# vita-epfl/Stable-Video-Infinity

Measured on AMD Instinct MI355X. Metric: denoised latent frames/sec, Wan2.1-1.3B 81f@832x480 50-step, higher is better.
Workload: dtype bf16

## Files before the change

include/svi_hip.h:

```cpp
#ifndef SVI_HIP_H
#define SVI_HIP_H

#include <stdint.h>

#ifdef __cplusplus
extern "C" {
#endif

#define SVI_HIP_ABI_VERSION 13

typedef enum {
    SVI_OK = 0,
    SVI_ERR_INVALID = 1,
    SVI_ERR_UNBOUND = 2,
    SVI_ERR_HIP = 3,
    SVI_ERR_UNSUPPORTED = 4,
    SVI_ERR_OOM = 5
} svi_status;

typedef enum { SVI_BF16 = 0, SVI_F32 = 1, SVI_F16 = 2 ,
               SVI_E4M3 = 3  } svi_dtype;

typedef void* svi_stream;
typedef struct svi_dit svi_dit;
// ... 32 lines not shown

svi_status svi_dit_forward(svi_dit* h, const void* x, const float* timestep, const void* context,
                           const void* clip_feature, const void* y, const void* add_condition,
                           void* out, int32_t B, int32_t T, int32_t H, int32_t W, int32_t Lc,
                           svi_stream stream);

svi_status svi_dit_set_audio(svi_dit* h, const void* audio_first, const void* audio_latter, int32_t n_latter);

svi_status svi_dit_audio_slot(svi_dit* h, int32_t slot , const void* audio_first, const void* audio_latter, int32_t n_latter,
                              svi_stream stream);
svi_status svi_dit_forward_talk3(svi_dit* h, const void* x, const float* timestep, const void* context_cond, const void* context_uncond,
                                 const void* clip_feature, const void* y, const void* add_condition, void* out_cond, void* out_uncond,
                                 void* out_drop_text, int32_t T, int32_t H, int32_t W, int32_t Lc, svi_stream stream);
svi_status svi_audio_windows(const void* emb, svi_dtype dtype, int32_t N, int32_t R, int32_t start, int32_t T_latent, void* first_out,
                             void* latter_out, svi_stream stream);
svi_status svi_dit_audio_slot_windows(svi_dit* h, int32_t slot , const void* emb, svi_dtype dtype, int32_t N, int32_t start,
                                      int32_t T_latent, svi_stream stream);
svi_status svi_dit_forward_talk3_tea(svi_dit* h, const void* x, const float* timestep, const void* context_cond, const void* context_uncond,
                                     const void* clip_feature, const void* y, const void* add_condition, void* out_cond, void* out_uncond,
                                     void* out_drop_text, int32_t T, int32_t H, int32_t W, int32_t Lc, int32_t tea_cond, int32_t tea_uncond,
                                     int32_t tea_drop_text, void* residual_cond, void* residual_uncond, void* residual_drop_text, svi_stream stream);

svi_status svi_dit_time_mod(svi_dit* h, const float* timestep, void* t_mod_out, int32_t B, svi_stream stream);
svi_status svi_dit_forward_tea(svi_dit* h, const void* x, const float* timestep, const void* context,
                               const void* clip_feature, const void* y, const void* add_condition, void* out,
                               int32_t B, int32_t T, int32_t H, int32_t W, int32_t Lc, int32_t tea_mode, void* residual,
                               svi_stream stream);

svi_status svi_dit_forward_cfg_pair(svi_dit* h, const void* x, const float* timestep, const void* context_cond,
                                    const void* context_uncond, const void* clip_feature, const void* y,
                                    const void* add_condition, void* out_cond, void* out_uncond, int32_t B, int32_t T,
                                    int32_t H, int32_t W, int32_t Lc, svi_stream stream);
svi_status svi_dit_forward_cfg_pair_tea(svi_dit* h, const void* x, const float* timestep, const void* context_cond,
                                        const void* context_uncond, const void* clip_feature, const void* y,
                                        const void* add_condition, void* out_cond, void* out_uncond, int32_t B, int32_t T,
                                        int32_t H, int32_t W, int32_t Lc, int32_t tea_mode, void* residual_cond, void* residual_uncond,
                                        svi_stream stream);

svi_status svi_dit_context_cache(svi_dit* h, int32_t enable);
svi_status svi_dit_context_refill(svi_dit* h, const void* context, const void* clip_feature, int32_t Lc, svi_stream stream);

svi_status svi_dit_sp_begin(svi_dit* h, const void* x, const float* timestep, const void* context, const void* clip_feature,
                            const void* y, const void* add_condition, int32_t T, int32_t H, int32_t W, int32_t Lc,
                            int32_t row0, int32_t nrows, svi_stream stream);
svi_status svi_dit_sp_begin_pair(svi_dit* h, const void* x, const float* timestep, const void* context_cond, const void* context_uncond,
                                 const void* clip_feature, const void* y, const void* add_condition, int32_t T, int32_t H, int32_t W, int32_t Lc,
                                 int32_t row0, int32_t nrows, svi_stream stream);
svi_status svi_dit_sp_block_qkv_part(svi_dit* h, int32_t layer, void* q_send, void* k_send, void* vt_out, int32_t ldvt, int32_t P, int32_t G,
                                     int32_t part, svi_stream stream);
svi_status svi_dit_sp_block_qkv(svi_dit* h, int32_t layer, void* q_send, void* k_send, void* vt_out, int32_t ldvt, int32_t P, int32_t G,
                                svi_stream stream);
svi_status svi_sp_unpack_vt(const void* recv, void* out, int32_t P, int32_t Dp, int32_t Ls, int32_t lds, int32_t L8, int32_t nb, int32_t Dg, svi_stream stream);
svi_status svi_sp_unpack_out(const void* recv, void* out, int32_t P, int32_t G, int32_t Ls, int32_t Dg, int32_t nb, svi_stream stream);
svi_status svi_dit_sp_block_rest(svi_dit* h, int32_t layer, const void* attn, svi_stream stream);
svi_status svi_dit_sp_tea(svi_dit* h, int32_t mode, void* residual, svi_stream stream);
svi_status svi_dit_sp_head(svi_dit* h, void* head_rows_out, svi_stream stream);
svi_status svi_dit_unpatchify(svi_dit* h, const void* head_rows, void* out, int32_t T, int32_t H, int32_t W, svi_stream stream);
int32_t svi_dit_head_ld(svi_dit* h);
int64_t svi_dit_generation(svi_dit* h);
svi_status svi_stream_buffers_release(svi_stream stream, int32_t all_streams);
svi_status svi_attention_vt_fwd(const void* q, int32_t ldq, const void* k, int32_t ldk, const void* vt, int32_t ldvt, void* out,
                                int32_t ldo, int32_t s_q, int32_t s_kv, int32_t n, int32_t q_prescaled, svi_stream stream);
svi_status svi_attention_frames_fwd(const void* q, int32_t ldq, const void* k, int32_t ldk, const void* vt, int32_t ldvt, void* out, int32_t ldo,
                                    int32_t row0, int32_t nrows, int32_t rows_per_frame, int32_t keys_per_frame, int32_t n, svi_stream stream);

svi_status svi_linear_row_stats(const void* A, int32_t lda, const void* W, int32_t ldw, void* C, int32_t ldc, int32_t M, int32_t N, int32_t K,
                                const void* bias, float eps, float* row_sumsq, int32_t ldss, float* rs_out, svi_stream stream);
svi_status svi_cross_attention_fwd(const void* q, int32_t ldq, const void* k, int32_t ldk, const void* vt, int32_t ldvt, void* out, int32_t ldo,
                                   int32_t s_q, int32_t s_kv, int32_t n, const int32_t* key_tail, const float* q_rs, const void* q_gain,
                                   float q_out_scale, svi_stream stream);

svi_status svi_dit_block_forward(svi_dit* h, int32_t layer, void* x_inout, const void* context,
                                 const void* t_mod, int32_t f, int32_t hh, int32_t ww, int32_t Lc,
                                 svi_stream stream);

svi_status svi_attention_fwd(const void* q, const void* k, const void* v, void* out, int32_t b,
                             int32_t s_q, int32_t s_kv, int32_t n, int32_t d, svi_stream stream);
svi_status svi_attention_last_flagged(svi_stream stream, int32_t* flagged_out, int32_t* workgroups_out);
svi_status svi_gemm_plan(int32_t M, int32_t N, int32_t K, int32_t epilogue, int32_t skinny, int32_t compute_units, int32_t* kernel_out);
svi_status svi_gemm_w8_plan(int32_t M, int32_t N, int32_t K, int32_t epilogue, int32_t skinny, int32_t compute_units, int32_t* kernel_out);
svi_status svi_attention_plan(int32_t s_q, int32_t s_kv, int32_t heads, int32_t compute_units, int32_t* out4);
svi_status svi_vae_conv_plan(int32_t Cin, int32_t Cout, int32_t kt, int32_t frames, int32_t Ho, int32_t Wo, int64_t* out8);
svi_status svi_vae_tile_order(int32_t ord_T, int32_t ord_Lf, int32_t ord_G, int64_t* out);

svi_status svi_layernorm_modulate(const void* x, void* out, int32_t rows, int32_t dim, float eps,
                                  const void* w, const void* b, const void* shift, const void* scale,
                                  svi_stream stream);

svi_status svi_rmsnorm_rope(void* x, int32_t ld, int32_t rows, int32_t dim, const void* weight, float eps,
                            int32_t rope, int32_t num_heads, int32_t f, int32_t h, int32_t w,
                            svi_stream stream);

svi_status svi_rmsnorm_rope_qk(void* x, int32_t ld, int32_t rows, int32_t dim, const void* weight_q, const void* weight_k,
                               float eps, float out_scale_q, float out_scale_k, int32_t rope,
                               int32_t f, int32_t h, int32_t w, int32_t row0, int32_t period, svi_stream stream);

svi_status svi_gemm_bf16(const void* A, int32_t lda, const void* W, int32_t ldw, void* C, int32_t ldc,
                         int32_t M, int32_t N, int32_t K, const void* bias, int32_t bias_along_m,
                         int32_t epilogue, const float* gate, const void* res, int32_t ldres,
                         svi_stream stream);
svi_status svi_gemm_bf16_pair(const void* A, int32_t lda, const void* W, int32_t ldw, void* C, int32_t ldc,
                              int32_t M, int32_t N, int32_t K, const void* bias, int32_t bias_along_m,
                              int32_t epilogue, const float* gate, const void* res, int32_t ldres,
                              const void* W2, const void* bias2, int32_t n_split, int32_t sel_m, int32_t sel_n,
                              svi_stream stream);
svi_status svi_gemm_bf16_skinny(const void* A, int32_t lda, const void* W, int32_t ldw, void* C, int32_t ldc, int32_t M, int32_t N, int32_t K,
                                const void* bias, int32_t epilogue, const float* gate, const void* res, int32_t ldres, int32_t w8, svi_stream stream);
svi_status svi_gemm_bf16_w8(const void* A, int32_t lda, const void* W8, int32_t ldw, void* C, int32_t ldc,
                            int32_t M, int32_t N, int32_t K, const void* bias, int32_t bias_along_m,
                            int32_t epilogue, const float* gate, const void* res, int32_t ldres,
                            const void* W2_8, const void* bias2, int32_t n_split, int32_t sel_m, int32_t sel_n,
                            svi_stream stream);

svi_status svi_mx8_quantize(const void* x, int32_t ldx, int32_t rows, int32_t K, void* q, int32_t ldq, void* scales, int32_t sc_rows, svi_stream stream);
svi_status svi_gemm_mx8(const void* A8, int32_t lda, const void* a_scales, int32_t sc_rows, const void* W8, int32_t ldw, void* C, int32_t ldc,
                        int32_t M, int32_t N, int32_t K, const void* bias, int32_t epilogue, const float* gate, const void* res, int32_t ldres,
                        svi_stream stream);
svi_status svi_dit_bind_ffn_fp8(svi_dit* h, int32_t layer, int32_t which, const void* e4m3_weight);
svi_status svi_dit_ffn_mx8(svi_dit* h, int32_t enable);
svi_status svi_gemm_mx8_wscaled(const void* A8, int32_t lda, const void* W8, int32_t ldw, const void* w_scales, int32_t sc_rows, void* C, int32_t ldc,
                                int32_t M, int32_t N, int32_t K, const void* bias, int32_t bias_along_m, svi_stream stream);
svi_status svi_dit_proj_mx8(svi_dit* h, int32_t enable);

svi_status svi_cfg_step(void* latents, const void* cond, const void* uncond, int64_t n, float cfg_scale,
                        float dsigma, svi_stream stream);

svi_status svi_cfg3_step(void* latents, const void* cond, const void* uncond, const void* drop_text, int64_t n, float s_text,
                         float s_audio, float dsigma, svi_stream stream);

svi_status svi_fp8_e4m3_to_bf16(const void* in, void* out, int64_t n, svi_stream stream);

svi_status svi_f32_to_fp8_e4m3(const void* in, svi_dtype in_dtype, void* out, int64_t n, svi_stream stream);

svi_status svi_lora_merge_e4m3(void* w8, int32_t out_f, int32_t in_f, const void* up, const void* down_t, svi_dtype dtype, int32_t r, float alpha,
                               svi_stream stream);

svi_status svi_prof_enable(int32_t on);
svi_status svi_prof_summary(char* buf, int64_t buflen);
svi_status svi_prof_select(const char* tags);

svi_status svi_vae_create(svi_vae** out);
svi_status svi_vae_destroy(svi_vae* h);
svi_status svi_vae_bind_weight(svi_vae* h, const char* name, const void* dev_ptr, svi_dtype dtype,
                               const int64_t* shape, int32_t rank);
svi_status svi_vae_check_bound(svi_vae* h);
svi_status svi_video_to_u8(const float* video, uint8_t* frames, int32_t T, int32_t H, int32_t W, svi_stream stream);
svi_status svi_u8_to_video(const uint8_t* frames, float* video, int32_t n, int32_t H, int32_t W, svi_stream stream);

svi_status svi_vae_decode(svi_vae* h, const float* latents, float* video, int32_t T, int32_t hh, int32_t ww,
                          svi_stream stream);
svi_status svi_vae_encode(svi_vae* h, const float* video, float* latents, int32_t T, int32_t H, int32_t W,
                          svi_stream stream);

svi_status svi_vae_tiled_decode(svi_vae* h, const float* latents, float* video, int32_t T, int32_t hh, int32_t ww,
                                int32_t size_h, int32_t size_w, int32_t stride_h, int32_t stride_w, svi_stream stream);
svi_status svi_vae_tiled_encode(svi_vae* h, const float* video, float* latents, int32_t T, int32_t H, int32_t W,
                                int32_t size_h, int32_t size_w, int32_t stride_h, int32_t stride_w, svi_stream stream);

svi_status svi_vae_split_plan(int32_t hh, int32_t ww, int32_t parts_h, int32_t parts_w, int32_t part, int32_t* out24);
svi_status svi_vae_decode_part(svi_vae* h, const float* latents, float* video, int32_t T, int32_t hh, int32_t ww, int32_t parts_h, int32_t parts_w,
                               int32_t part, int32_t video_ld_h, int32_t video_ld_w, svi_stream stream);
svi_status svi_vae_decode_planned(svi_vae* h, const float* latents, float* video, int32_t T, int32_t hh, int32_t ww, const int32_t* plan24,
                                  int32_t video_ld_h, int32_t video_ld_w, svi_stream stream);

svi_status svi_vae_encode_split_plan(int32_t hh, int32_t ww, int32_t parts_h, int32_t parts_w, int32_t part, int32_t* out34);
svi_status svi_vae_encode_part(svi_vae* h, const float* video, float* feat_out, int32_t T, int32_t H, int32_t W, int32_t parts_h, int32_t parts_w,
// ... 63 lines not shown
```

stable-video-infinity_amd/csrc/svi_api.hip:

```cpp
#include <algorithm>
#include <string>
#include <stdlib.h>
#include <string.h>
#include <atomic>
#include <deque>
#include <mutex>
#include <vector>

#include "svi_common.h"

static thread_local char g_err[512] = "";

void svi_set_error(const char* fmt, ...) {
    va_list ap;
    va_start(ap, fmt);
    vsnprintf(g_err, sizeof(g_err), fmt, ap);
    va_end(ap);
}

extern "C" const char* svi_last_error(void) { return g_err; }

static int env_int(const char* name, int lo, int dflt) {
    const char* v = getenv(name);
    if (!v || !*v) return dflt;
    char* end = nullptr;
    const long x = strtol(v, &end, 10);
    if (end == v || x < lo || x > (1 << 20)) { fprintf(stderr, "libsvi_hip: ignoring %s=%s (expected an integer >= %d)\n", name, v, lo); return dflt; }
    return (int)x;
}
static SviSwitches parse_switches() {
    SviSwitches s;
    s.flash_kernel = env_int("SVI_FLASH_KERNEL", 1, 0);
    if (s.flash_kernel > 2) s.flash_kernel = 0;
    s.gemm_kernel = env_int("SVI_GEMM_KERNEL", 128, 0);
    if (s.gemm_kernel != 128 && s.gemm_kernel != 192 && s.gemm_kernel != 259 && s.gemm_kernel != 260) {
        if (s.gemm_kernel != 0)
            fprintf(stderr, "libsvi_hip: ignoring SVI_GEMM_KERNEL=%d (kernels: 128, 192, 259 = 256^2 four phases, 260 = 256^2 two phases; 256 / 257 / 258 are retired)\n", s.gemm_kernel);
        s.gemm_kernel = 0;
    }
    s.gemm_gm = env_int("SVI_GEMM_GM", 1, 0);
    s.gemm_pf = env_int("SVI_GEMM_PF", 1, 0);
    if (s.gemm_pf != 0 && s.gemm_pf != 1 && s.gemm_pf != 4 && s.gemm_pf != 8) s.gemm_pf = 0;
    s.vae_exact_fp32 = getenv("SVI_VAE_EXACT_FP32") != nullptr;
    s.flash_two_pass = env_int("SVI_FLASH_TWO_PASS", 0, 1);
    s.flash_m16 = env_int("SVI_FLASH_M16", 0, 1);
    s.vae_no_x2h = env_int("SVI_VAE_X2H", 0, 1) == 0;
    s.cross_dedup = env_int("SVI_CROSS_DEDUP", 0, 1);
    s.cross_fused = env_int("SVI_CROSS_FUSED", 0, 1);
    s.vae_dma = env_int("SVI_VAE_DMA", 0, 1);
    s.vae_up_phases = env_int("SVI_VAE_UP_PHASES", 0, 1);
    s.vae_tile_order = env_int("SVI_VAE_TILE_ORDER", 0, 1);
    s.vae_pair = env_int("SVI_VAE_PAIR", 0, 1);
    s.mx8_fused = env_int("SVI_MX8_FUSED", 0, 1);
    s.qk_fused = env_int("SVI_QK_FUSED", 0, 1);
    s.attn_qk8 = env_int("SVI_ATTN_QK8", 0, 0) != 0;
    s.qk8_fused = env_int("SVI_QK8_FUSED", 0, 1);
    s.rms_rows = env_int("SVI_RMS_ROWS", 0, 1);
    s.flash_split = env_int("SVI_FLASH_SPLIT", 0, 0);
    if (s.flash_split > 4) s.flash_split = 4;
    s.ws_limit_mb = env_int("SVI_WS_LIMIT_MB", 1, 0);
    { const char* v = getenv("SVI_T5_BUCKETS"); s.t5_host_buckets = v && strcmp(v, "host") == 0; }
    return s;
}
static std::atomic<const SviSwitches*>& switches_ptr() {
    static std::atomic<const SviSwitches*> p{new SviSwitches(parse_switches())};
    return p;
}
const SviSwitches& svi_switches() { return *switches_ptr().load(std::memory_order_acquire); }
static std::atomic<unsigned long long> g_stream_buffer_generation{0};
extern "C" svi_status svi_switches_reload(void) {
    switches_ptr().store(new SviSwitches(parse_switches()), std::memory_order_release);
    g_stream_buffer_generation.fetch_add(1, std::memory_order_relaxed);
    return SVI_OK;
}

extern "C" int32_t svi_switch_state(const char* name) {
    if (!name) return -1;
    const SviSwitches& sw = svi_switches();
    const std::string n(name);
    if (n == "SVI_ATTN_QK8") return sw.attn_qk8 ? 1 : 0;
    if (n == "SVI_CROSS_FUSED") return sw.cross_fused ? 1 : 0;
    if (n == "SVI_CROSS_DEDUP") return sw.cross_dedup ? 1 : 0;
    if (n == "SVI_QK_FUSED") return sw.qk_fused ? 1 : 0;
    if (n == "SVI_FLASH_TWO_PASS") return sw.flash_two_pass ? 1 : 0;
    if (n == "SVI_FLASH_M16") return sw.flash_m16 ? 1 : 0;
    return -1;
}

int svi_current_device() {
    int d = -1;
    if (hipGetDevice(&d) != hipSuccess) { (void)hipGetLastError(); svi_set_error("no usable HIP device"); return -1; }
    return d;
}

svi_status svi_claim_device(int* handle_device) {
    const int d = svi_current_device();
    if (d < 0) return SVI_ERR_HIP;
    if (*handle_device < 0) *handle_device = d;
    if (*handle_device != d) {
        svi_set_error("handle belongs to device %d but the current device is %d (one handle per device)", *handle_device, d);
        return SVI_ERR_INVALID;
    }
    return SVI_OK;
}

static std::mutex& table_mutex() {
    static std::mutex m;
    return m;
}

svi_status svi_ensure_lds(const void* kernel, int bytes) {
    struct Seen { int dev; const void* fn; };
    static std::vector<Seen> seen;
    const int dev = svi_current_device();
    if (dev < 0) return SVI_ERR_HIP;
    std::lock_guard<std::mutex> lock(table_mutex());
    for (const Seen& s : seen)
        if (s.dev == dev && s.fn == kernel) return SVI_OK;
    SVI_CHECK_HIP(hipFuncSetAttribute(kernel, hipFuncAttributeMaxDynamicSharedMemorySize, bytes));
    seen.push_back(Seen{dev, kernel});
    return SVI_OK;
}

namespace {
struct StreamSlot { int dev, kind; hipStream_t st; void* p; size_t bytes; long user; };
std::deque<StreamSlot>& stream_slots() {
    static std::deque<StreamSlot> slots;
    return slots;
}
}
unsigned long long svi_stream_buffer_generation() { return g_stream_buffer_generation.load(std::memory_order_relaxed); }

extern "C" svi_status svi_stream_buffers_release(svi_stream stream, int32_t all_streams) {
    const int dev = svi_current_device();
    if (dev < 0) return SVI_ERR_HIP;
// ... 339 lines not shown
    g.C = reinterpret_cast<bf16*>(C); g.ldc = ldc; g.M = M; g.N = N; g.K = K;
    g.bias = reinterpret_cast<const bf16*>(bias); g.bias_along_m = bias_along_m; g.epi = epilogue; g.gate = gate;
    g.res = reinterpret_cast<const bf16*>(res); g.ldres = ldres;
    if (W2) { g.W2 = reinterpret_cast<const bf16*>(W2); g.bias2 = reinterpret_cast<const bf16*>(bias2); g.n_split = n_split; }
    g.sel_m = sel_m; g.sel_n = sel_n;
    return svi_launch_gemm_e8(g, 1, reinterpret_cast<hipStream_t>(stream));
}

extern "C" svi_status svi_gemm_bf16_skinny(const void* A, int32_t lda, const void* W, int32_t ldw, void* C, int32_t ldc, int32_t M, int32_t N, int32_t K,
                                           const void* bias, int32_t epilogue, const float* gate, const void* res, int32_t ldres, int32_t w8, svi_stream stream) {
    SVI_REQUIRE(A && W && C, "svi_gemm_bf16_skinny: null argument");
    SviGemmArgs g{};
    g.A = reinterpret_cast<const bf16*>(A); g.lda = lda; g.W = reinterpret_cast<const bf16*>(W); g.ldw = ldw;
    g.C = reinterpret_cast<bf16*>(C); g.ldc = ldc; g.M = M; g.N = N; g.K = K;
    g.bias = reinterpret_cast<const bf16*>(bias); g.epi = epilogue; g.gate = gate; g.res = reinterpret_cast<const bf16*>(res); g.ldres = ldres;
    g.skinny = 1;
    SVI_REQUIRE(svi_gemm_choose(g, 256) == 0, "svi_gemm_bf16_skinny: M = %d, K = %d, epilogue %d do not take the skinny kernel (M <= 128, K %% 128 == 0, bias or gate + residual)", M, K, epilogue);
    return w8 ? svi_launch_gemm_e8(g, 1, reinterpret_cast<hipStream_t>(stream)) : svi_launch_gemm(g, reinterpret_cast<hipStream_t>(stream));
}

extern "C" svi_status svi_linear_row_stats(const void* A, int32_t lda, const void* W, int32_t ldw, void* C, int32_t ldc, int32_t M, int32_t N, int32_t K,
                                           const void* bias, float eps, float* row_sumsq, int32_t ldss, float* rs_out, svi_stream stream) {
    SVI_REQUIRE(A && W && C && row_sumsq && rs_out, "svi_linear_row_stats: null argument");
    SVI_REQUIRE(N > 0 && N % 64 == 0 && ldss >= M, "svi_linear_row_stats: N = %d must be a multiple of 64 and ldss >= M", N);
    hipStream_t st = reinterpret_cast<hipStream_t>(stream);
    SviGemmArgs g{};
    g.A = reinterpret_cast<const bf16*>(A); g.lda = lda; g.W = reinterpret_cast<const bf16*>(W); g.ldw = ldw;
    g.C = reinterpret_cast<bf16*>(C); g.ldc = ldc; g.M = M; g.N = N; g.K = K;
    g.bias = reinterpret_cast<const bf16*>(bias); g.epi = SVI_EPI_BIAS;
    g.rowss = row_sumsq; g.ldss = ldss;
    SVI_TRY(svi_launch_gemm(g, st));
    return svi_launch_row_rs(row_sumsq, N / 64, ldss, M, N, eps, rs_out, st);
}
extern "C" svi_status svi_cross_attention_fwd(const void* q, int32_t ldq, const void* k, int32_t ldk, const void* vt, int32_t ldvt, void* out, int32_t ldo,
                                              int32_t s_q, int32_t s_kv, int32_t n, const int32_t* key_tail, const float* q_rs, const void* q_gain,
                                              float q_out_scale, svi_stream stream) {
    SVI_REQUIRE(q && k && vt && out, "svi_cross_attention_fwd: null argument");
    SVI_REQUIRE(s_q > 0 && s_kv > 0 && n > 0 && ldq >= n * 128 && ldk >= n * 128 && ldo >= n * 128 && ldvt >= s_kv, "svi_cross_attention_fwd: bad sizes");
    SVI_REQUIRE((q_rs == nullptr) == (q_gain == nullptr), "svi_cross_attention_fwd: q_rs and q_gain come together");
    hipStream_t st = reinterpret_cast<hipStream_t>(stream);
    SviProfScope _p(PROF_FLASH_CROSS, st);
    const SviQNorm qn{q_rs, reinterpret_cast<const bf16*>(q_gain), q_out_scale};
    int key_blocks = 0;
    if (key_tail) {
        hipStreamCaptureStatus cs = hipStreamCaptureStatusNone;
        int n = 0;
        if (hipStreamIsCapturing(st, &cs) == hipSuccess && cs == hipStreamCaptureStatusNone &&
            hipMemcpyAsync(&n, key_tail, sizeof(int), hipMemcpyDeviceToHost, st) == hipSuccess && hipStreamSynchronize(st) == hipSuccess && n > 0)
            key_blocks = (std::min(n, s_kv) + 31) / 32;
        else (void)hipGetLastError();
    }
    return svi_launch_flash_cross(reinterpret_cast<const bf16*>(q), ldq, reinterpret_cast<const bf16*>(k), ldk, reinterpret_cast<const bf16*>(vt), ldvt,
                                  reinterpret_cast<bf16*>(out), ldo, s_q, s_kv, n, st, key_tail, q_rs ? &qn : nullptr, key_blocks);
}

extern "C" svi_status svi_gemm_plan(int32_t M, int32_t N, int32_t K, int32_t epilogue, int32_t skinny, int32_t compute_units, int32_t* kernel_out) {
    SVI_REQUIRE(kernel_out && M > 0 && N > 0 && K > 0 && compute_units > 0, "svi_gemm_plan: bad argument");
    SviGemmArgs g{};
    g.M = M; g.N = N; g.K = K; g.lda = K; g.ldw = K; g.ldc = (N + 7) / 8 * 8; g.epi = epilogue; g.skinny = skinny;
    *kernel_out = svi_gemm_choose(g, compute_units);
    return SVI_OK;
}
extern "C" svi_status svi_gemm_w8_plan(int32_t M, int32_t N, int32_t K, int32_t epilogue, int32_t skinny, int32_t compute_units, int32_t* kernel_out) {
    SVI_REQUIRE(kernel_out && M > 0 && N > 0 && K > 0 && compute_units > 0, "svi_gemm_w8_plan: bad argument");
    SviGemmArgs g{};
    g.M = M; g.N = N; g.K = K; g.lda = K; g.ldw = K; g.ldc = (N + 7) / 8 * 8; g.epi = epilogue; g.skinny = skinny;
    *kernel_out = svi_gemm_choose_e8(g, compute_units, 1);
    return SVI_OK;
}
extern "C" svi_status svi_attention_plan(int32_t s_q, int32_t s_kv, int32_t heads, int32_t compute_units, int32_t* out4) {
    SVI_REQUIRE(out4 && s_q > 0 && s_kv > 0 && heads > 0 && compute_units > 0, "svi_attention_plan: bad argument");
    int kernel = 0;
    const SviFlashSplit sp = svi_flash_plan(s_q, s_kv, heads, compute_units, &kernel);
    const int items = sp.qblocks * sp.heads;
    out4[0] = kernel; out4[1] = sp.whole; out4[2] = sp.pieces; out4[3] = sp.whole + (items - sp.whole) * sp.pieces;
    return SVI_OK;
}
extern "C" svi_status svi_vae_conv_plan(int32_t Cin, int32_t Cout, int32_t kt, int32_t frames, int32_t Ho, int32_t Wo, int64_t* out8) {
    return svi_vae_conv_choose(Cin, Cout, kt, frames, Ho, Wo, out8);
}
extern "C" svi_status svi_vae_tile_order(int32_t ord_T, int32_t ord_Lf, int32_t ord_G, int64_t* out) {
    return svi_vae_tile_order_fill(ord_T, ord_Lf, ord_G, out);
}

extern "C" svi_status svi_mx8_quantize(const void* x, int32_t ldx, int32_t rows, int32_t K, void* q, int32_t ldq, void* scales, int32_t sc_rows,
                                       svi_stream stream) {
    SVI_REQUIRE(x && q && scales, "svi_mx8_quantize: null argument");
    return svi_launch_mx8_quantize(reinterpret_cast<const bf16*>(x), ldx, rows, K, reinterpret_cast<unsigned char*>(q), ldq, reinterpret_cast<unsigned*>(scales), sc_rows,
                                   reinterpret_cast<hipStream_t>(stream));
}
extern "C" svi_status svi_gemm_mx8(const void* A8, int32_t lda, const void* a_scales, int32_t sc_rows, const void* W8, int32_t ldw, void* C, int32_t ldc,
                                   int32_t M, int32_t N, int32_t K, const void* bias, int32_t epilogue, const float* gate, const void* res, int32_t ldres,
                                   svi_stream stream) {
    SVI_REQUIRE(A8 && a_scales && W8 && C, "svi_gemm_mx8: null argument");
    SviGemmArgs g{};
    g.A = reinterpret_cast<const bf16*>(A8); g.lda = lda; g.W = reinterpret_cast<const bf16*>(W8); g.ldw = ldw;
    g.C = reinterpret_cast<bf16*>(C); g.ldc = ldc; g.M = M; g.N = N; g.K = K;
    g.bias = reinterpret_cast<const bf16*>(bias); g.epi = epilogue; g.gate = gate; g.res = reinterpret_cast<const bf16*>(res); g.ldres = ldres;
    return svi_launch_gemm_mx8(g, reinterpret_cast<const unsigned*>(a_scales), sc_rows, reinterpret_cast<hipStream_t>(stream));
}

extern "C" svi_status svi_gemm_mx8_wscaled(const void* A8, int32_t lda, const void* W8, int32_t ldw, const void* w_scales, int32_t sc_rows, void* C, int32_t ldc,
                                           int32_t M, int32_t N, int32_t K, const void* bias, int32_t bias_along_m, svi_stream stream) {
    SVI_REQUIRE(A8 && w_scales && W8 && C, "svi_gemm_mx8_wscaled: null argument");
    SviGemmArgs g{};
    g.A = reinterpret_cast<const bf16*>(A8); g.lda = lda; g.W = reinterpret_cast<const bf16*>(W8); g.ldw = ldw;
    g.C = reinterpret_cast<bf16*>(C); g.ldc = ldc; g.M = M; g.N = N; g.K = K;
    g.bias = reinterpret_cast<const bf16*>(bias); g.bias_along_m = bias_along_m; g.epi = SVI_EPI_BIAS;
    return svi_launch_gemm_mx8_wscaled(g, reinterpret_cast<const unsigned*>(w_scales), sc_rows, reinterpret_cast<hipStream_t>(stream));
}

extern "C" svi_status svi_cfg_step(void* latents, const void* cond, const void* uncond, int64_t n, float cfg_scale,
                                   float dsigma, svi_stream stream) {
    SVI_REQUIRE(latents && cond, "svi_cfg_step: null argument");
    return svi_launch_cfg_step(reinterpret_cast<bf16*>(latents), reinterpret_cast<const bf16*>(cond),
                               reinterpret_cast<const bf16*>(uncond), n, cfg_scale, dsigma,
                               reinterpret_cast<hipStream_t>(stream));
}

extern "C" svi_status svi_fp8_e4m3_to_bf16(const void* in, void* out, int64_t n, svi_stream stream) {
    SVI_REQUIRE(in && out && n >= 0, "svi_fp8_e4m3_to_bf16: bad argument");
    return svi_launch_fp8_e4m3_to_bf16(reinterpret_cast<const unsigned char*>(in), reinterpret_cast<bf16*>(out), n, reinterpret_cast<hipStream_t>(stream));
}

extern "C" svi_status svi_cfg3_step(void* latents, const void* cond, const void* uncond, const void* drop_text, int64_t n, float s_text,
                                    float s_audio, float dsigma, svi_stream stream) {
    SVI_REQUIRE(latents && cond && uncond && drop_text && n >= 0, "svi_cfg3_step: bad argument");
    return svi_launch_cfg3_step(reinterpret_cast<bf16*>(latents), reinterpret_cast<const bf16*>(cond), reinterpret_cast<const bf16*>(uncond),
                                reinterpret_cast<const bf16*>(drop_text), n, s_text, s_audio, dsigma, reinterpret_cast<hipStream_t>(stream));
}

extern "C" svi_status svi_audio_windows(const void* emb, svi_dtype dtype, int32_t N, int32_t R, int32_t start, int32_t T_latent, void* first_out,
                                        void* latter_out, svi_stream stream) {
    SVI_REQUIRE(emb, "svi_audio_windows: emb is NULL");
    SVI_REQUIRE(dtype == SVI_F32 || dtype == SVI_BF16, "svi_audio_windows: emb must be fp32 or bf16 (dtype %d)", (int)dtype);
    SVI_REQUIRE(N >= 1, "svi_audio_windows: N = %d audio frames (at least one)", N);
    SVI_REQUIRE(T_latent >= 1, "svi_audio_windows: T_latent = %d (at least one latent frame)", T_latent);
    SVI_REQUIRE(R > 0 && R % 8 == 0, "svi_audio_windows: R = %d must be a positive multiple of 8", R);
    SVI_REQUIRE(start >= 0, "svi_audio_windows: start = %d is negative", start);
    SVI_REQUIRE(first_out && (T_latent == 1 || latter_out), "svi_audio_windows: NULL output");
    if (svi_current_device() < 0) return SVI_ERR_HIP;
    return svi_launch_audio_windows(emb, dtype == SVI_F32, N, R, start, T_latent, reinterpret_cast<bf16*>(first_out), reinterpret_cast<bf16*>(latter_out),
                                    reinterpret_cast<hipStream_t>(stream));
}
```

stable-video-infinity_amd/csrc/svi_common.h:

```cpp
#pragma once

#include <hip/hip_runtime.h>
#include <stdint.h>
#include <stdarg.h>
#include <stdio.h>

#include "../../include/svi_hip.h"

typedef __bf16 bf16;
typedef __attribute__((ext_vector_type(8))) __bf16 bf16x8;
typedef __attribute__((ext_vector_type(4))) __bf16 bf16x4;
typedef __attribute__((ext_vector_type(2))) __bf16 bf16x2;
typedef __attribute__((ext_vector_type(16))) float f32x16;
typedef __attribute__((ext_vector_type(4))) float f32x4;
typedef __attribute__((ext_vector_type(4))) unsigned int u32x4;
typedef __attribute__((ext_vector_type(2))) unsigned int u32x2;

#define SVI_WAVE 64

void svi_set_error(const char* fmt, ...);

#define SVI_CHECK_HIP(expr)                                                                   \
    do {                                                                                      \
        hipError_t _e = (expr);                                                               \
        if (_e != hipSuccess) {                                                               \
            svi_set_error("%s failed: %s (%s:%d)", #expr, hipGetErrorString(_e), __FILE__, __LINE__); \
            return SVI_ERR_HIP;                                                               \
        }                                                                                     \
    } while (0)

#define SVI_REQUIRE(cond, ...)                                                                \
    do {                                                                                      \
        if (!(cond)) {                                                                        \
            svi_set_error(__VA_ARGS__);                                                       \
            return SVI_ERR_INVALID;                                                           \
        }                                                                                     \
    } while (0)

#define SVI_LAUNCH_CHECK()                                                                    \
    do {                                                                                      \
        hipError_t _e = hipGetLastError();                                                    \
        if (_e != hipSuccess) {                                                               \
            svi_set_error("kernel launch failed: %s (%s:%d)", hipGetErrorString(_e), __FILE__, __LINE__); \
            return SVI_ERR_HIP;                                                               \
        }                                                                                     \
    } while (0)

#define SVI_TRY(expr)                                                                         \
    do {                                                                                      \
        svi_status _s = (expr);                                                               \
        if (_s != SVI_OK) return _s;                                                          \
    } while (0)

struct SviSwitches {
    int flash_kernel = 0;
    int gemm_kernel = 0;
    int gemm_pf = 0;
    int gemm_gm = 0;
    int vae_exact_fp32 = 0;
    int vae_no_x2h = 0;
    int vae_dma = 1;
    int vae_pair = 1;
    int vae_tile_order = 1;
    int vae_up_phases = 1;
    int flash_two_pass = 1;
    int flash_m16 = 1;
    int flash_split = 0;
    int rms_rows = 1;
    int qk_fused = 1;
    int mx8_fused = 1;
    int attn_qk8 = 0;
    int qk8_fused = 1;
    int cross_fused = 1;
    int cross_dedup = 1;
    int t5_host_buckets = 0;
    int ws_limit_mb = 0;
};
const SviSwitches& svi_switches();

svi_status svi_ensure_lds(const void* kernel, int bytes);
enum SviBufKind { SVI_BUF_FLASH_FLAGS = 0, SVI_BUF_SEAM_SCRATCH = 1, SVI_BUF_SEAM_SMALL = 2, SVI_BUF_FLASH_SPLIT = 3, SVI_BUF_FLASH_QK8 = 4 };
svi_status svi_stream_buffer(int kind, hipStream_t st, size_t bytes, void** out, long** user_out);
int svi_current_device();
svi_status svi_claim_device(int* handle_device);
#define SVI_REQUIRE_DEVICE(h) SVI_TRY(svi_claim_device(&(h)->device))

#ifdef __HIPCC__
__device__ __forceinline__ float rbf(float v) { return (float)(bf16)v; }

__device__ __forceinline__ float wave_sum(float v) {
#pragma unroll
    for (int o = 32; o > 0; o >>= 1) v += __shfl_xor(v, o);
    return v;
}
__device__ __forceinline__ float wave_max(float v) {
#pragma unroll
    for (int o = 32; o > 0; o >>= 1) v = fmaxf(v, __shfl_xor(v, o));
    return v;
}

__device__ __forceinline__ bf16x8 ld_bf16x8(const bf16* p) { return *reinterpret_cast<const bf16x8*>(p); }
__device__ __forceinline__ void st_bf16x8(bf16* p, bf16x8 v) { *reinterpret_cast<bf16x8*>(p) = v; }

__device__ __forceinline__ void mx8_quant8(const float (&v)[8], bool live, int row, int c8, unsigned char* __restrict__ q, int ldq,
                                           unsigned* __restrict__ scales, int sc_rows) {
    float amax = 0.f;
#pragma unroll
    for (int e = 0; e < 8; ++e) amax = fmaxf(amax, fabsf(v[e]));
    amax = fmaxf(amax, __shfl_xor(amax, 1));
    amax = fmaxf(amax, __shfl_xor(amax, 2));
    const int eb = (int)((__float_as_uint(amax) >> 23) & 0xffu);
    const int E = max(eb - 8, 0);
    const float inv = __uint_as_float((unsigned)(254 - E) << 23);
    unsigned w[2];
#pragma unroll
    for (int h2 = 0; h2 < 2; ++h2) {
        float a[4];
#pragma unroll
        for (int e = 0; e < 4; ++e) {
            const float t = v[4 * h2 + e] * inv;
            a[e] = t != t ? t : fminf(fmaxf(t, -448.f), 448.f);
        }
        unsigned pk = 0;
        pk = __builtin_amdgcn_cvt_pk_fp8_f32(a[0], a[1], pk, false);
        pk = __builtin_amdgcn_cvt_pk_fp8_f32(a[2], a[3], pk, true);
        w[h2] = pk;
    }
    if (live) *reinterpret_cast<u32x2*>(q + (size_t)row * ldq + c8 * 8) = u32x2{w[0], w[1]};
    const int lane = threadIdx.x & 63;
    const unsigned e0 = (unsigned)E;
    const unsigned e1 = (unsigned)__shfl(E, (lane & ~15) + 4), e2 = (unsigned)__shfl(E, (lane & ~15) + 8), e3 = (unsigned)__shfl(E, (lane & ~15) + 12);
    if (live && (lane & 15) == 0) scales[(size_t)(c8 >> 4) * sc_rows + row] = e0 | (e1 << 8) | (e2 << 16) | (e3 << 24);
}

__device__ __forceinline__ float gelu_tanh_f(float x) {
    const float A = -2.0f * 1.4426950408889634f * 0.7978845608028654f * 0.044715f, B = -2.0f * 1.4426950408889634f * 0.7978845608028654f;
    const float a = x * __builtin_fmaf(x * x, A, B);
    return x * __builtin_amdgcn_rcpf(1.0f + __builtin_amdgcn_exp2f(a));
}
__device__ __forceinline__ float gelu_erf_f(float x) { return 0.5f * x * (1.0f + erff(x * 0.7071067811865476f)); }
__device__ __forceinline__ float silu_f(float x) { return x / (1.0f + __expf(-x)); }
#endif

enum SviProfTag {
    PROF_LN = 0, PROF_GEMM_QKV, PROF_RMS_ROPE, PROF_FLASH_SELF, PROF_GEMM_O, PROF_GEMM_CROSS, PROF_FLASH_CROSS,
    PROF_GEMM_FFN1, PROF_GEMM_FFN2, PROF_EMBED, PROF_HEAD, PROF_VAE_CONV, PROF_VAE_OTHER, PROF_NTAGS
};
extern bool g_svi_prof_on;
extern unsigned g_svi_prof_mask;
void svi_prof_begin_impl(int tag, hipStream_t st);
void svi_prof_end_impl(int tag, hipStream_t st);
struct SviProfScope {
    int tag; hipStream_t st; bool on;
    SviProfScope(int t, hipStream_t s) : tag(t), st(s), on(g_svi_prof_on && ((g_svi_prof_mask >> t) & 1u)) { if (on) svi_prof_begin_impl(tag, st); }
    ~SviProfScope() { if (on) svi_prof_end_impl(tag, st); }
};

struct SviGemmArgs {
    const bf16* A; int lda;
    const bf16* W; int ldw;
    bf16* C; int ldc;
    int M, N, K;
    const bf16* bias; int bias_along_m;
    int epi;
    const float* gate;
    const bf16* res; int ldres;
    int sel_m, sel_n;
    int skinny;
    unsigned char* q8; int ldq8; unsigned* q8s; int q8_sc_rows;
    const bf16* W2; const bf16* bias2; int n_split;
    float* rowss; int ldss;
};
unsigned long long svi_stream_buffer_generation();
svi_status svi_launch_gemm(const SviGemmArgs& g, hipStream_t st);
int svi_gemm_choose(const SviGemmArgs& g, int compute_units);
svi_status svi_launch_gemm_e8(const SviGemmArgs& g, int e8, hipStream_t st);
int svi_gemm_choose_e8(const SviGemmArgs& g, int compute_units, int e8);
struct SviFlashSplit { int whole, pieces, qblocks, heads; };
SviFlashSplit svi_flash_plan(int Lq, int Lk, int heads, int cus, int* kernel_out);
svi_status svi_vae_conv_choose(int Cin, int Cout, int kt, int frames, int Ho, int Wo, int64_t* out8);
svi_status svi_vae_tile_order_fill(int ord_T, int ord_Lf, int ord_G, int64_t* out);
svi_status svi_launch_mx8_quantize(const bf16* x, int ldx, int rows, int K, unsigned char* q, int ldq, unsigned* scales, int sc_rows, hipStream_t st);
svi_status svi_launch_gemm_mx8(const SviGemmArgs& g, const unsigned* a_scales, int sc_rows, hipStream_t st);
svi_status svi_launch_gemm_mx8_wscaled(const SviGemmArgs& g, const unsigned* w_scales, int sc_rows, hipStream_t st);

#define SVI_QK_SCALE_LOG2E 0.12751743f
struct SviQk8 { unsigned char* q8; unsigned char* k8; unsigned* qs; unsigned* ks; int ld8, qs_rows, ks_rows; };
svi_status svi_launch_flash(const bf16* Q, int ldq, const bf16* K, int ldk, const bf16* VT, int ldvt,
                            bf16* O, int ldo, int Lq, int Lk, int num_heads, int q_prescaled, hipStream_t st, const int* key_tail = nullptr, const SviQk8* qk8 = nullptr);
svi_status svi_launch_flash_frames(const bf16* Q, int ldq, const bf16* K, int ldk, const bf16* VT, int ldvt, bf16* O, int ldo, int row0, int nrows,
                                   int rows_per_frame, int keys_per_frame, int num_heads, hipStream_t st);
struct SviQNorm { const float* rs; const bf16* gain; float out_scale; };
svi_status svi_launch_flash_cross(const bf16* Q, int ldq, const bf16* K, int ldk, const bf16* VT, int ldvt, bf16* O, int ldo, int Lq, int Lk, int num_heads,
                                  hipStream_t st, const int* key_tail, const SviQNorm* norm, int key_blocks = 0);
svi_status svi_launch_row_rs(const float* rowss, int groups, int ldss, int rows, int dim, float eps, float* rs, hipStream_t st);
svi_status svi_flash_qk8_prepare(int Lq, int Lk, int num_heads, hipStream_t st, SviQk8* out, bool* use, int batch = 1);
inline SviQk8 svi_qk8_sample(const SviQk8& b, int s, int Lq, int Lk) {
    SviQk8 v = b;
    v.q8 += (size_t)s * Lq * b.ld8; v.k8 += (size_t)s * Lk * b.ld8; v.qs += (size_t)s * Lq; v.ks += (size_t)s * Lk;
    return v;
}

svi_status svi_launch_ln_mod(const bf16* x, int ldx, bf16* out, int ldo, int rows, int dim, float eps,
                             const bf16* w, const bf16* b, const float* shift, const float* scale1p,
                             hipStream_t st);
struct SviRope {
    const float2* tab_f; const float2* tab_h; const float2* tab_w;
    int npf, nph, npw;
    int f, h, w;
    int row0;
    int period;
    const float2* tab_tok;
};
svi_status svi_launch_rope_token_table(const SviRope& r, float2* out, int tokens, hipStream_t st);
struct SviScatter { bf16* out0; bf16* out1; int P, Dp, Dg; int rows_per_sample; };
svi_status svi_launch_rmsnorm_rope(bf16* x, int ld, int rows, int dim, const bf16* weight, float eps,
                                   const SviRope* rope, float out_scale, hipStream_t st);
svi_status svi_launch_rmsnorm_rope2(bf16* x, int ld, int rows, int dim, const bf16* weight, const bf16* weight1, float eps,
                                    const SviRope* rope, float out_scale, float out_scale1, hipStream_t st, const SviScatter* scatter = nullptr);
bool svi_rmsnorm_rope_q8_ok(int dim, const SviRope* rope);
svi_status svi_launch_rmsnorm_rope2_q8(bf16* x, int ld, int rows, int dim, const bf16* weight, const bf16* weight1, float eps, const SviRope* rope, float out_scale,
                                       float out_scale1, hipStream_t st, const SviQk8& out);
svi_status svi_launch_sp_unpack_vt(const bf16* recv, bf16* out, int P, int Dp, int Ls, int lds, int L8, hipStream_t st, int nb = 1, int Dg = 0);
svi_status svi_launch_sp_unpack_out(const bf16* recv, bf16* out, int P, int G, int Ls, int Dg, hipStream_t st, int nb = 1);
svi_status svi_launch_transpose(const bf16* in, int ldi, bf16* out, int ldo, int rows, int cols, hipStream_t st);
svi_status svi_launch_cfg_step(bf16* lat, const bf16* cond, const bf16* uncond, int64_t n, float s, float dsigma,
                               hipStream_t st);
svi_status svi_launch_add_bf16(bf16* a_inout, const bf16* b, int64_t n, hipStream_t st);
svi_status svi_launch_cfg3_step(bf16* lat, const bf16* cond, const bf16* uncond, const bf16* drop, int64_t n, float st, float sa, float dsigma,
                                hipStream_t stream);
svi_status svi_launch_video_to_u8(const float* video, unsigned char* out, long thw, hipStream_t st);
svi_status svi_launch_u8_to_video(const unsigned char* frames, float* out, int n, long hw, hipStream_t st);
svi_status svi_launch_sub_bf16(bf16* out, const bf16* a, const bf16* b, int64_t n, hipStream_t st);
svi_status svi_launch_audio_windows(const void* emb, bool f32, int N, int R, int start, int T, bf16* first, bf16* latter, hipStream_t st);
svi_status svi_launch_add_ln_mod_pair(const bf16* x, const bf16* res_a, const bf16* res_b, bf16* out_a, bf16* out_b, int rows, int dim, float eps,
                                      const float* shift, const float* scale1p, hipStream_t st);
svi_status svi_launch_sub_sum_bf16(bf16* out, const bf16* a, const bf16* b, const bf16* c, int64_t n, hipStream_t st);
svi_status svi_launch_add_ln_mod_talk3(const bf16* x, const bf16* add_condition, const bf16* const res[3], bf16* const out[3], const bool with_addc[3],
                                       int rows, int dim, float eps, const float* shift, const float* scale1p, hipStream_t st);
svi_status svi_launch_fp8_e4m3_to_bf16(const unsigned char* in, bf16* out, int64_t n, hipStream_t st);
svi_status svi_launch_gemm_f32(const float* A, int lda, const float* W, int ldw, const float* bias, float* C, int ldc, int M, int N, int K,
                               const float* res, int ldres, hipStream_t st);
```

stable-video-infinity_amd/csrc/svi_vae.hip:

```cpp
#include <algorithm>
#include <map>
#include <string>
#include <vector>
#include <math.h>
#include <stdlib.h>
#include <string.h>

#include "svi_common.h"

namespace {

struct ConvP {
    const float* in; int Ti, Hi, Wi, Cin, ld_in;
    const float* w; int ld_w;
    const bf16* w3; int ld_w3; long plane_w3;
    const void* w2h; const float* w2_inv;
    float in_scale;
    const float* bias;
    float* out; int To, Ho, Wo, Cout, ld_out;
    int kt, kh, kw, st, sh, sw, pt, ph, pw;
    int ups;
    int zero_frame0;
    int t_begin;
    int out_mode;
    int pad_;
    int t_out_off;
    const float* res; int ld_res;
    int act_silu;
    bf16* out_bf16;
    const unsigned short* in_h; const unsigned short* in_l;
    int ord_T, ord_Lf, ord_G;
    int up_phase;
};

__device__ __forceinline__ int tile_off(int row, int chunk) { return row * 128 + ((chunk ^ ((row >> 1) & 7)) << 4); }

template <int NT>
__global__ __launch_bounds__(256, 2) void conv_igemm_kernel(ConvP p) {
    constexpr int A_BYTES = 128 * 128;
    constexpr int W_BYTES = NT * 32 * 128;
    extern __shared__ __attribute__((aligned(16))) char smem[];
    const int tid = threadIdx.x, lane = tid & 63, wave = tid >> 6;
    const int l31 = lane & 31, hi = lane >> 5;
    const long HoWo = (long)p.Ho * p.Wo;
    const long P_total = (long)p.To * HoWo;
    const long p0 = (long)p.t_begin * HoWo + (long)blockIdx.x * 128;
    const int co0 = blockIdx.y * 32 * NT;
    const int Hv = p.ups ? 2 * p.Hi : p.Hi, Wv = p.ups ? 2 * p.Wi : p.Wi;

    const int ld_chunk = tid & 7;
    int a_t[4], a_y[4], a_x[4];
    bool a_ok[4];
#pragma unroll
    for (int j = 0; j < 4; ++j) {
        const long pp = p0 + (tid >> 3) + 32 * j;
        a_ok[j] = pp < P_total;
        const long q = a_ok[j] ? pp : 0;
        a_t[j] = (int)(q / HoWo);
        const int rem = (int)(q - (long)a_t[j] * HoWo);
        a_y[j] = rem / p.Wo;
        a_x[j] = rem - a_y[j] * p.Wo;
    }
    const int nchunk = (p.Cin + 31) >> 5;
    const int ntaps = p.kt * p.kh * p.kw;
    const int nk = ntaps * nchunk;
    f32x4 ra[4], rw[NT];
    const f32x4 zero4 = {0.f, 0.f, 0.f, 0.f};

    auto load_tile = [&](int kidx) {
        const int tap = kidx / nchunk, cc = kidx - tap * nchunk;
        const int ta = tap / (p.kh * p.kw), tb = (tap / p.kw) % p.kh, tc = tap % p.kw;
        const int c = cc * 32 + ld_chunk * 4;
        const bool cin = c < p.Cin;
#pragma unroll
        for (int j = 0; j < 4; ++j) {
            const int ti = a_t[j] * p.st + ta - p.pt;
            int yi = a_y[j] * p.sh + tb - p.ph, xi = a_x[j] * p.sw + tc - p.pw;
            bool ok = a_ok[j] && cin && ti >= 0 && ti < p.Ti && yi >= 0 && yi < Hv && xi >= 0 && xi < Wv;
            if (p.zero_frame0 && ti == 0) ok = false;
            if (p.ups) { yi >>= 1; xi >>= 1; }
            ra[j] = ok ? *reinterpret_cast<const f32x4*>(p.in + (((long)ti * p.Hi + yi) * p.Wi + xi) * p.ld_in + c) : zero4;
        }
#pragma unroll
        for (int j = 0; j < NT; ++j) {
            const int co = co0 + (tid >> 3) + 32 * j;
            rw[j] = (cin && co < p.Cout) ? *reinterpret_cast<const f32x4*>(p.w + ((long)tap * p.Cout + co) * p.ld_w + c) : zero4;
        }
    };
    auto store_tile = [&](int buf) {
        char* As = smem + buf * (A_BYTES + W_BYTES);
        char* Ws = As + A_BYTES;
#pragma unroll
        for (int j = 0; j < 4; ++j) *reinterpret_cast<f32x4*>(As + tile_off((tid >> 3) + 32 * j, ld_chunk)) = ra[j];
#pragma unroll
        for (int j = 0; j < NT; ++j) *reinterpret_cast<f32x4*>(Ws + tile_off((tid >> 3) + 32 * j, ld_chunk)) = rw[j];
    };

    f32x16 acc[NT];
#pragma unroll
    for (int n = 0; n < NT; ++n)
#pragma unroll
        for (int r = 0; r < 16; ++r) acc[n][r] = 0.f;

    load_tile(0);
    store_tile(0);
    __syncthreads();
    for (int k = 0; k < nk; ++k) {
        const int cur = k & 1;
        if (k + 1 < nk) load_tile(k + 1);
        const char* As = smem + cur * (A_BYTES + W_BYTES);
        const char* Ws = As + A_BYTES;
#pragma unroll
        for (int q = 0; q < 4; ++q) {
            const f32x4 av = *reinterpret_cast<const f32x4*>(As + tile_off(32 * wave + l31, 2 * q + hi));
            f32x4 bv[NT];
// ... 366 lines not shown
    for (int k = 0; k < nk; k += 2) {
        SVI_X3_STEP(0, 0, k + 2, k + 2 < nk, 1, 1);
        __syncthreads();
        SVI_X3_STEP(1, 1, k + 3, k + 3 < nk, 0, 0);
        __syncthreads();
    }
#undef SVI_X3_STEP
#undef SVI_X3_ADVANCE
#undef SVI_X3_TAP_BASES
#undef SVI_X3_LOAD_A
#undef SVI_X3_LOAD_W
#undef SVI_X3_STAGE_A
#undef SVI_X3_STAGE_W
#undef SVI_X3_SPLIT1
#undef SVI_X3_MFMA
#undef SVI_X3_STORES
#undef SVI_X3_LOADS

    const long pp = p0 + 32 * wave + l31;
    if (pp >= P_total) return;
    const f32x4 zero4 = {0.f, 0.f, 0.f, 0.f};
    f32x4 bv[12], rv[12], sv[12];
    const bool with_res = p.out_mode == 0 && p.res;
    const float inv_a = H2 ? 1.0f / p.in_scale : 1.0f;
    long po = pp + (long)p.t_out_off * HoWo;
    if (!H2 && p.up_phase) {
        const int ph_ = p.up_phase - 1;
        const int t = (int)(pp / HoWo);
        const int rem = (int)(pp - (long)t * HoWo);
        const int y = rem / p.Wo, x = rem - y * p.Wo;
        po = ((long)(t + p.t_out_off) * (2 * p.Ho) + 2 * y + (ph_ >> 1)) * (2 * p.Wo) + 2 * x + (ph_ & 1);
    }
#pragma unroll
    for (int i = 0; i < 12; ++i) {
        const int co = co0 + 32 * (i >> 2) + 8 * (i & 3) + 4 * hi;
        const bool ok = co < p.Cout;
        bv[i] = (ok && p.bias) ? *reinterpret_cast<const f32x4*>(p.bias + co) : zero4;
        rv[i] = (ok && with_res) ? *reinterpret_cast<const f32x4*>(p.res + po * p.ld_res + co) : zero4;
        if constexpr (H2) sv[i] = ok ? *reinterpret_cast<const f32x4*>(p.w2_inv + co) * inv_a : zero4;
    }
    long pq0 = 0;
    const int half = p.Cout >> 1;
    if (p.out_mode != 0) {
        const int t = (int)(pp / HoWo);
        const long sp = pp - (long)t * HoWo;
        pq0 = (long)(1 + 2 * (t - 1)) * HoWo + sp;
    }
#pragma unroll
    for (int i = 0; i < 12; ++i) {
        const int n = i >> 2, rg = i & 3;
        const int co = co0 + 32 * n + 8 * rg + 4 * hi;
        if (co >= p.Cout) continue;
        f32x4 v;
#pragma unroll
        for (int e = 0; e < 4; ++e) {
            float a = acc[n][4 * rg + e];
            if constexpr (H2) a *= sv[i][e];
            v[e] = (a + bv[i][e]) + rv[i][e];
        }
        if (p.out_mode == 0) {
            *reinterpret_cast<f32x4*>(p.out + po * p.ld_out + co) = v;
        } else {
            const int j = co >= half ? 1 : 0;
            *reinterpret_cast<f32x4*>(p.out + (pq0 + (long)j * HoWo) * p.ld_out + (co - j * half)) = v;
        }
    }
}


#define D2_ROWS 272
__host__ __device__ __forceinline__ long conv_tile_at(int ord_T, int ord_Lf, int ord_G, long tile) {
    if (ord_T <= 0) return tile;
    const long per_group = (long)ord_T * ord_G;
    const int full = ord_Lf / ord_G;
    const long g = tile / per_group;
    int gl = ord_G;
    long r = tile - g * per_group, gbase = g * ord_G;
    if (g >= full) { gl = ord_Lf - full * ord_G; r = tile - (long)full * per_group; gbase = (long)full * ord_G; }
    const int t = (int)(r / gl), j = (int)(r - (long)t * gl);
    return (long)t * ord_Lf + gbase + j;
}
#define D2_A_PLANE (D2_ROWS * 64)
#define D2_STAGE (2 * D2_A_PLANE + 6 * X3_W_PLANE)
template <int NB>
__global__ __launch_bounds__(512, 2) void conv_dma2h_kernel(ConvP p) {
#ifdef SVI_D2_DENSE
    p.ld_in = 32; p.ld_w3 = 32;
#endif
    constexpr int WP = 2 * NB;
    constexpr int NPIECE = 34 + 6 * WP;
    constexpr int D2_SLOTS = (NPIECE + 7) / 8;
    extern __shared__ __attribute__((aligned(16))) char smem[];
    const int tid = threadIdx.x, lane = tid & 63;
    const int wave = __builtin_amdgcn_readfirstlane(tid >> 6);
    const int l31 = lane & 31, hi = lane >> 5;
    const long HoWo = (long)p.Ho * p.Wo;
    const long P_total = (long)p.To * HoWo;
    const int ncob = (p.Cout + NB * 32 - 1) / (NB * 32);
    long tile = blockIdx.x / ncob;
    const int cob = (int)(blockIdx.x - tile * ncob);
    if (p.ord_T > 0) tile = conv_tile_at(p.ord_T, p.ord_Lf, p.ord_G, tile);
    const long p0 = (long)p.t_begin * HoWo + tile * X3_PIX;
    const int co0 = cob * NB * 32;
    const int nchunk = p.Cin >> 5;
    const int nrow = p.kt * p.kh;
    const int nk = nrow * nchunk;

    const int t_first = (int)(max(min(p0 - 1, P_total - 1), 0L) / HoWo);
    const int t_base = max(t_first * p.st - p.pt, 0);
    unsigned s_off[D2_SLOTS], s_mask[D2_SLOTS];
#pragma unroll
    for (int i = 0; i < D2_SLOTS; ++i) {
        const int q = wave + 8 * i;
        s_off[i] = 0xFFF00000u; s_mask[i] = 0;
        if (q < 34) {
            const int r16 = q % 17, row = r16 * 16 + (lane >> 2);
            const long pp = p0 - 1 + row;
            const bool pix = pp >= 0 && pp < P_total;
            const long qq = pix ? pp : 0;
            const int at = (int)(qq / HoWo);
            const int rem = (int)(qq - (long)at * HoWo);
            const int ay = rem / p.Wo, ax = rem - ay * p.Wo;
            const int bt = at * p.st - p.pt, by = ay - p.ph;
            unsigned m = 0;
            for (int rt = 0; rt < nrow; ++rt) {
                const int ta = rt / p.kh, tb = rt - ta * p.kh;
                const int ti = bt + ta, yi = by + tb;
                bool ok = pix && ti >= 0 && ti < p.Ti && yi >= 0 && yi < p.Hi;
                if (p.zero_frame0 && ti == 0) ok = false;
                if (ok) m |= 1u << rt;
            }
            s_mask[i] = m;
            const int chunk = (lane & 3) ^ ((row >> 2) & 3);
            s_off[i] = (unsigned)((((bt - t_base) * p.Hi + by) * p.Wi + ax) * p.ld_in) * 2u + (unsigned)chunk * 16u;
        } else if (q < NPIECE) {
            const int w = q - 34, tc = w / (2 * WP), pl = (w % (2 * WP)) / WP, row = (w % WP) * 16 + (lane >> 2);
            const int chunk = (lane & 3) ^ ((row >> 2) & 3);
            if (co0 + row < p.Cout) s_off[i] = (unsigned)((pl * p.plane_w3 + ((long)tc * p.Cout + co0 + row) * p.ld_w3 + chunk * 8) * 2);
        }
    }
    const long base_el = (long)t_base * p.Hi * p.Wi * p.ld_in;
    const long rem_bytes = ((long)p.Ti * p.Hi * p.Wi * p.ld_in - base_el) * 2;
    const int win = (int)(unsigned)min(rem_bytes, 0xFFE00000L);
    const __amdgpu_buffer_rsrc_t rs_h = __builtin_amdgcn_make_buffer_rsrc(const_cast<unsigned short*>(p.in_h + base_el), 0, win, 0x00020000);
    const __amdgpu_buffer_rsrc_t rs_l = __builtin_amdgcn_make_buffer_rsrc(const_cast<unsigned short*>(p.in_l + base_el), 0, win, 0x00020000);
    const __amdgpu_buffer_rsrc_t rs_w = __builtin_amdgcn_make_buffer_rsrc(const_cast<void*>(p.w2h), 0, (int)(unsigned)min((long)2 * p.plane_w3 * 2, 0xFFE00000L), 0x00020000);
    const unsigned OOB = 0xFFF00000u;
    bool left_ok, right_ok;
    {
        const long pp = min(p0 + 32 * wave + l31, P_total - 1);
        const int ax = (int)(pp % p.Wo);
        left_ok = ax > 0; right_ok = ax < p.Wo - 1;
    }

    int it_rt = 0, it_cc = 0, it_ta = 0, it_tb = 0;
    auto request = [&](int buf) {
        char* As = smem + buf * D2_STAGE;
        char* Ws = As + 2 * D2_A_PLANE;
        const unsigned d_act = (unsigned)(((it_ta * p.Hi + it_tb) * p.Wi) * p.ld_in) * 2u + (unsigned)it_cc * 64u;
        const unsigned d_w = (unsigned)((long)it_rt * p.kw * p.Cout * p.ld_w3 * 2) + (unsigned)it_cc * 64u;
#pragma unroll
        for (int i = 0; i < D2_SLOTS; ++i) {
            const int q = wave + 8 * i;
            if (q < 34) {
#ifdef SVI_D2_SKIP_A
                if (it_rt | it_cc) continue;
#endif
                const int pl = q / 17, r16 = q % 17;
                const unsigned off = ((s_mask[i] >> it_rt) & 1u) ? s_off[i] + d_act : OOB;
                if (pl == 0) __builtin_amdgcn_raw_ptr_buffer_load_lds(rs_h, (lptr_t)(As + r16 * 1024), 16, off, 0, 0, 0);
                else __builtin_amdgcn_raw_ptr_buffer_load_lds(rs_l, (lptr_t)(As + D2_A_PLANE + r16 * 1024), 16, off, 0, 0, 0);
            } else if (q < NPIECE) {
#ifdef SVI_D2_SKIP_W
                if (it_rt | it_cc) continue;
#endif
                const int w = q - 34, tc = w / (2 * WP), pl = (w % (2 * WP)) / WP, r16 = w % WP;
                const unsigned off = s_off[i] == OOB ? OOB : s_off[i] + d_w;
                __builtin_amdgcn_raw_ptr_buffer_load_lds(rs_w, (lptr_t)(Ws + (tc * 2 + pl) * X3_W_PLANE + r16 * 1024), 16, off, 0, 0, 0);
            }
        }
    };
    auto advance = [&]() {
        if (++it_cc == nchunk) {
            it_cc = 0; ++it_rt;
            if (++it_tb == p.kh) { it_tb = 0; ++it_ta; }
        }
    };

    f32x16 acc[NB];
#pragma unroll
    for (int n = 0; n < NB; ++n)
#pragma unroll
        for (int r = 0; r < 16; ++r) acc[n][r] = 0.f;

    request(0);
    advance();
    __syncthreads();
    const f16x8 zero8 = {(f16)0, (f16)0, (f16)0, (f16)0, (f16)0, (f16)0, (f16)0, (f16)0};
    for (int k = 0; k < nk; ++k) {
        const int cur = k & 1;
        if (k + 1 < nk) request(cur ^ 1);
        advance();
        const char* As = smem + cur * D2_STAGE;
        const char* Ws = As + 2 * D2_A_PLANE;
        f16x8 ah[2], al[2], wh[2][NB], wl[2][NB];
        auto frags = [&](int sidx, int set) {
            const int tc = sidx >> 1, ks = sidx & 1;
            const bool live = tc == 0 ? left_ok : tc == 2 ? right_ok : true;
            f16x8 h_ = *reinterpret_cast<const f16x8*>(As + x3_off(32 * wave + l31 + tc, 2 * ks + hi));
            f16x8 l_ = *reinterpret_cast<const f16x8*>(As + D2_A_PLANE + x3_off(32 * wave + l31 + tc, 2 * ks + hi));
            if (tc != 1) { h_ = live ? h_ : zero8; l_ = live ? l_ : zero8; }
            ah[set] = h_; al[set] = l_;
#pragma unroll
            for (int n = 0; n < NB; ++n) {
                wh[set][n] = *reinterpret_cast<const f16x8*>(Ws + (tc * 2) * X3_W_PLANE + x3_off(32 * n + l31, 2 * ks + hi));
                wl[set][n] = *reinterpret_cast<const f16x8*>(Ws + (tc * 2 + 1) * X3_W_PLANE + x3_off(32 * n + l31, 2 * ks + hi));
            }
        };
        frags(0, 0);
#pragma unroll
        for (int sidx = 0; sidx < 6; ++sidx) {
            const int set = sidx & 1;
            if (sidx + 1 < 6) frags(sidx + 1, set ^ 1);
#pragma unroll
            for (int n = 0; n < NB; ++n) acc[n] = __builtin_amdgcn_mfma_f32_32x32x16_f16(wl[set][n], ah[set], acc[n], 0, 0, 0);
#pragma unroll
            for (int n = 0; n < NB; ++n) acc[n] = __builtin_amdgcn_mfma_f32_32x32x16_f16(wh[set][n], al[set], acc[n], 0, 0, 0);
#pragma unroll
            for (int n = 0; n < NB; ++n) acc[n] = __builtin_amdgcn_mfma_f32_32x32x16_f16(wh[set][n], ah[set], acc[n], 0, 0, 0);
        }
        __syncthreads();
    }

    const long pp = p0 + 32 * wave + l31;
    if (pp >= P_total) return;
    const f32x4 zero4 = {0.f, 0.f, 0.f, 0.f};
    f32x4 bv[4 * NB], rv[4 * NB], sv[4 * NB];
    const bool with_res = p.out_mode == 0 && p.res;
    const float inv_a = 1.0f / p.in_scale;
    const long po = pp + (long)p.t_out_off * HoWo;
#pragma unroll
    for (int i = 0; i < 4 * NB; ++i) {
        const int co = co0 + 32 * (i >> 2) + 8 * (i & 3) + 4 * hi;
        const bool ok = co < p.Cout;
        if (NB == 1 && ok && co + 4 > p.Cout) {
            bv[i] = zero4; sv[i] = zero4; rv[i] = zero4;
            for (int e = 0; e < 4; ++e)
                if (co + e < p.Cout) {
                    if (p.bias) bv[i][e] = p.bias[co + e];
                    sv[i][e] = p.w2_inv[co + e] * inv_a;
                    if (with_res) rv[i][e] = p.res[po * p.ld_res + co + e];
                }
            continue;
        }
        bv[i] = (ok && p.bias) ? *reinterpret_cast<const f32x4*>(p.bias + co) : zero4;
        rv[i] = (ok && with_res) ? *reinterpret_cast<const f32x4*>(p.res + po * p.ld_res + co) : zero4;
        sv[i] = ok ? *reinterpret_cast<const f32x4*>(p.w2_inv + co) * inv_a : zero4;
    }
    long pq0 = 0;
    const int half = p.Cout >> 1;
    if (p.out_mode != 0) {
        const int t = (int)(pp / HoWo);
        const long sp = pp - (long)t * HoWo;
        pq0 = (long)(1 + 2 * (t - 1)) * HoWo + sp;
    }
#pragma unroll
    for (int i = 0; i < 4 * NB; ++i) {
        const int n = i >> 2, rg = i & 3;
        const int co = co0 + 32 * n + 8 * rg + 4 * hi;
        if (co >= p.Cout) continue;
        f32x4 v;
#pragma unroll
        for (int e = 0; e < 4; ++e) v[e] = (acc[n][4 * rg + e] * sv[i][e] + bv[i][e]) + rv[i][e];
        if (p.out_mode == 0) {
            *reinterpret_cast<f32x4*>(p.out + po * p.ld_out + co) = v;
        } else {
            const int j = co >= half ? 1 : 0;
            *reinterpret_cast<f32x4*>(p.out + (pq0 + (long)j * HoWo) * p.ld_out + (co - j * half)) = v;
        }
    }
}

#define D2P_W_STAGE (6 * X3_W_PLANE)
#define D2P_LDS (2 * D2P_W_STAGE + 2 * 2 * D2_A_PLANE)
__global__ __launch_bounds__(512, 2) void conv_dma2h_pair_kernel(ConvP p) {
    constexpr int NB = 3, WP = 2 * NB;
    constexpr int A_SLOTS = 5, W_SLOTS = 5;
    extern __shared__ __attribute__((aligned(16))) char smem[];
    char* const Wbuf = smem;
    char* const Sbuf = smem + 2 * D2P_W_STAGE;
    const int tid = threadIdx.x, lane = tid & 63;
    const int wave = __builtin_amdgcn_readfirstlane(tid >> 6);
    const int l31 = lane & 31, hi = lane >> 5;
    const long HoWo = (long)p.Ho * p.Wo;
    const long P_total = (long)p.To * HoWo;
    const int ncob = (p.Cout + NB * 32 - 1) / (NB * 32);
    const long pair = blockIdx.x / ncob;
    const int cob = (int)(blockIdx.x - pair * ncob);
    const int co0 = cob * NB * 32;
    const int nchunk = p.Cin >> 5;
    const int nrow = p.kt * p.kh;
    const int nk = nrow * nchunk;
    const unsigned OOB = 0xFFF00000u;

    long p0[2];
    int t_base[2];
#pragma unroll
    for (int s = 0; s < 2; ++s) {
        long tile = 2 * pair + s;
        if (tile < (long)p.ord_T * p.ord_Lf) tile = conv_tile_at(p.ord_T, p.ord_Lf, p.ord_G, tile);
        p0[s] = (long)p.t_begin * HoWo + tile * X3_PIX;
        const int t_first = (int)(max(min(p0[s] - 1, P_total - 1), 0L) / HoWo);
        t_base[s] = max(t_first * p.st - p.pt, 0);
    }
    unsigned a_off[2][A_SLOTS], a_mask[2][A_SLOTS], w_off[W_SLOTS];
#pragma unroll
    for (int s = 0; s < 2; ++s)
#pragma unroll
        for (int i = 0; i < A_SLOTS; ++i) {
            const int q = wave + 8 * i;
            a_off[s][i] = OOB; a_mask[s][i] = 0;
            if (q < 34) {
                const int r16 = q % 17, row = r16 * 16 + (lane >> 2);
                const long pp = p0[s] - 1 + row;
                const bool pix = pp >= 0 && pp < P_total;
                const long qq = pix ? pp : 0;
                const int at = (int)(qq / HoWo);
                const int rem = (int)(qq - (long)at * HoWo);
                const int ay = rem / p.Wo, ax = rem - ay * p.Wo;
                const int bt = at * p.st - p.pt, by = ay - p.ph;
                unsigned m = 0;
                for (int rt = 0; rt < nrow; ++rt) {
                    const int ta = rt / p.kh, tb = rt - ta * p.kh;
                    const int ti = bt + ta, yi = by + tb;
                    bool ok = pix && ti >= 0 && ti < p.Ti && yi >= 0 && yi < p.Hi;
                    if (p.zero_frame0 && ti == 0) ok = false;
                    if (ok) m |= 1u << rt;
                }
                a_mask[s][i] = m;
                const int chunk = (lane & 3) ^ ((row >> 2) & 3);
                a_off[s][i] = (unsigned)((((bt - t_base[s]) * p.Hi + by) * p.Wi + ax) * p.ld_in) * 2u + (unsigned)chunk * 16u;
            }
        }
#pragma unroll
    for (int i = 0; i < W_SLOTS; ++i) {
        const int w = wave + 8 * i;
        w_off[i] = OOB;
        if (w < 6 * WP) {
            const int tc = w / (2 * WP), pl = (w % (2 * WP)) / WP, row = (w % WP) * 16 + (lane >> 2);
            const int chunk = (lane & 3) ^ ((row >> 2) & 3);
            if (co0 + row < p.Cout) w_off[i] = (unsigned)((pl * p.plane_w3 + ((long)tc * p.Cout + co0 + row) * p.ld_w3 + chunk * 8) * 2);
        }
    }
    __amdgpu_buffer_rsrc_t rs_h[2], rs_l[2];
#pragma unroll
    for (int s = 0; s < 2; ++s) {
        const long base_el = (long)t_base[s] * p.Hi * p.Wi * p.ld_in;
        const long rem_bytes = ((long)p.Ti * p.Hi * p.Wi * p.ld_in - base_el) * 2;
        const int win = (int)(unsigned)min(rem_bytes, 0xFFE00000L);
        rs_h[s] = __builtin_amdgcn_make_buffer_rsrc(const_cast<unsigned short*>(p.in_h + base_el), 0, win, 0x00020000);
        rs_l[s] = __builtin_amdgcn_make_buffer_rsrc(const_cast<unsigned short*>(p.in_l + base_el), 0, win, 0x00020000);
    }
    const __amdgpu_buffer_rsrc_t rs_w = __builtin_amdgcn_make_buffer_rsrc(const_cast<void*>(p.w2h), 0, (int)(unsigned)min((long)2 * p.plane_w3 * 2, 0xFFE00000L), 0x00020000);
    bool left_ok[2], right_ok[2];
#pragma unroll
    for (int s = 0; s < 2; ++s) {
        const long pp = min(p0[s] + 32 * wave + l31, P_total - 1);
// ... 27 lines not shown
        char* Ws = Wbuf + wb * D2P_W_STAGE;
        const unsigned d_w = (unsigned)((long)rt * p.kw * p.Cout * p.ld_w3 * 2) + (unsigned)cc * 64u;
#pragma unroll
        for (int i = 0; i < W_SLOTS; ++i) {
            const int w = wave + 8 * i;
            if ((i < 2) != (half == 0) || w >= 6 * WP) continue;
            const int tc = w / (2 * WP), pl = (w % (2 * WP)) / WP, r16 = w % WP;
            const unsigned off = w_off[i] == OOB ? OOB : w_off[i] + d_w;
            __builtin_amdgcn_raw_ptr_buffer_load_lds(rs_w, (lptr_t)(Ws + (tc * 2 + pl) * X3_W_PLANE + r16 * 1024), 16, off, 0, 0, 0);
        }
    };

    f32x16 acc[2][NB];
#pragma unroll
    for (int s = 0; s < 2; ++s)
#pragma unroll
        for (int n = 0; n < NB; ++n)
#pragma unroll
            for (int r = 0; r < 16; ++r) acc[s][n][r] = 0.f;
    const f16x8 zero8 = {(f16)0, (f16)0, (f16)0, (f16)0, (f16)0, (f16)0, (f16)0, (f16)0};
    auto multiply = [&](auto sc, int wb) {
        constexpr int S = decltype(sc)::value;
        const char* As = Sbuf + S * 2 * D2_A_PLANE;
        const char* Ws = Wbuf + wb * D2P_W_STAGE;
        f16x8 ah[2], al[2], wh[2][NB], wl[2][NB];
        auto frags = [&](int sidx, int set) {
            const int tc = sidx >> 1, ks = sidx & 1;
            const bool live = tc == 0 ? left_ok[S] : tc == 2 ? right_ok[S] : true;
            f16x8 h_ = *reinterpret_cast<const f16x8*>(As + x3_off(32 * wave + l31 + tc, 2 * ks + hi));
            f16x8 l_ = *reinterpret_cast<const f16x8*>(As + D2_A_PLANE + x3_off(32 * wave + l31 + tc, 2 * ks + hi));
            if (tc != 1) { h_ = live ? h_ : zero8; l_ = live ? l_ : zero8; }
            ah[set] = h_; al[set] = l_;
#pragma unroll
            for (int n = 0; n < NB; ++n) {
                wh[set][n] = *reinterpret_cast<const f16x8*>(Ws + (tc * 2) * X3_W_PLANE + x3_off(32 * n + l31, 2 * ks + hi));
                wl[set][n] = *reinterpret_cast<const f16x8*>(Ws + (tc * 2 + 1) * X3_W_PLANE + x3_off(32 * n + l31, 2 * ks + hi));
            }
        };
        frags(0, 0);
#pragma unroll
        for (int sidx = 0; sidx < 6; ++sidx) {
            const int set = sidx & 1;
            if (sidx + 1 < 6) frags(sidx + 1, set ^ 1);
#pragma unroll
            for (int n = 0; n < NB; ++n) acc[S][n] = __builtin_amdgcn_mfma_f32_32x32x16_f16(wl[set][n], ah[set], acc[S][n], 0, 0, 0);
#pragma unroll
            for (int n = 0; n < NB; ++n) acc[S][n] = __builtin_amdgcn_mfma_f32_32x32x16_f16(wh[set][n], al[set], acc[S][n], 0, 0, 0);
#pragma unroll
            for (int n = 0; n < NB; ++n) acc[S][n] = __builtin_amdgcn_mfma_f32_32x32x16_f16(wh[set][n], ah[set], acc[S][n], 0, 0, 0);
        }
    };
    std::integral_constant<int, 0> T0;
    std::integral_constant<int, 1> T1;

    request_w(0, 0, 0, 0);
    request_w(1, 0, 0, 0);
    request_strip(T0, 0, 0, 0, 0);
    step_next(n_rt, n_cc, n_ta, n_tb);
    __syncthreads();
    for (int k = 0; k < nk; ++k) {
        const int wb = k & 1;
        const bool more = k + 1 < nk;
        request_strip(T1, c_rt, c_cc, c_ta, c_tb);
        if (more) request_w(0, n_rt, n_cc, wb ^ 1);
        multiply(T0, wb);
        __syncthreads();
        if (more) {
            request_strip(T0, n_rt, n_cc, n_ta, n_tb);
            request_w(1, n_rt, n_cc, wb ^ 1);
        }
        multiply(T1, wb);
        __syncthreads();
        step_next(c_rt, c_cc, c_ta, c_tb);
        step_next(n_rt, n_cc, n_ta, n_tb);
    }

    const f32x4 zero4 = {0.f, 0.f, 0.f, 0.f};
    const bool with_res = p.out_mode == 0 && p.res;
    const float inv_a = 1.0f / p.in_scale;
    const int half = p.Cout >> 1;
#pragma unroll
    for (int s = 0; s < 2; ++s) {
        const long pp = p0[s] + 32 * wave + l31;
        if (pp >= P_total) continue;
        const long po = pp + (long)p.t_out_off * HoWo;
        long pq0 = 0;
        if (p.out_mode != 0) {
            const int t = (int)(pp / HoWo);
            const long sp = pp - (long)t * HoWo;
            pq0 = (long)(1 + 2 * (t - 1)) * HoWo + sp;
        }
#pragma unroll
        for (int i = 0; i < 4 * NB; ++i) {
            const int n = i >> 2, rg = i & 3;
            const int co = co0 + 32 * n + 8 * rg + 4 * hi;
            if (co >= p.Cout) continue;
            const f32x4 bv = p.bias ? *reinterpret_cast<const f32x4*>(p.bias + co) : zero4;
            const f32x4 rv = with_res ? *reinterpret_cast<const f32x4*>(p.res + po * p.ld_res + co) : zero4;
            const f32x4 sv = *reinterpret_cast<const f32x4*>(p.w2_inv + co) * inv_a;
            f32x4 v;
#pragma unroll
            for (int e = 0; e < 4; ++e) v[e] = (acc[s][n][4 * rg + e] * sv[e] + bv[e]) + rv[e];
            if (p.out_mode == 0) {
                *reinterpret_cast<f32x4*>(p.out + po * p.ld_out + co) = v;
            } else {
                const int j = co >= half ? 1 : 0;
                *reinterpret_cast<f32x4*>(p.out + (pq0 + (long)j * HoWo) * p.ld_out + (co - j * half)) = v;
            }
        }
    }
}

bool conv_planes_ok(const ConvP& p) {
    const bool vec_ok = (((uintptr_t)p.w2_inv | (uintptr_t)p.bias) & 15) == 0;
    const bool wide = p.Cout >= 64 && p.Cout % 4 == 0 && vec_ok && (p.out_mode == 0 || (p.Cout / 2) % 4 == 0);
    const bool narrow = p.Cout <= 32 && p.out_mode == 0 && (p.Cout % 4 != 0 || vec_ok);
    return p.w2h && p.w2_inv && p.in_scale > 0.f && !svi_switches().vae_no_x2h && !svi_switches().vae_exact_fp32 && svi_switches().vae_dma &&
           p.Cin % 32 == 0 && p.ld_in == p.Cin && !p.ups && (wide || narrow) &&
           p.kw == 3 && p.kh == 3 && p.kt * p.kh <= 32 && p.st == 1 && p.sh == 1 && p.sw == 1 && p.ph == 1 && p.pw == 1 && p.Ho == p.Hi && p.Wo == p.Wi &&
           !p.act_silu && !p.out_bf16 &&
           (long)(p.kt + 3) * p.Hi * p.Wi * p.ld_in * 2 < 0xFFE00000L && (long)2 * p.plane_w3 * 2 < 0xFFE00000L;
}

struct ConvPlanesPlan {
    int kernel;
    int ord_T, ord_Lf, ord_G;
    long tiles, workgroups;
};
ConvPlanesPlan conv_planes_plan(const ConvP& p) {
    ConvPlanesPlan r{};
    const long hw = (long)p.Ho * p.Wo;
    const int frames = p.To - p.t_begin;
    r.tiles = (frames * hw + X3_PIX - 1) / X3_PIX;
    if (svi_switches().vae_tile_order && p.kt > 1 && frames > 1 && hw % X3_PIX == 0) {
        r.ord_T = frames; r.ord_Lf = (int)(hw / X3_PIX);
        r.ord_G = (int)std::max<long>(1, std::min<long>(r.ord_Lf, (16L * p.Wo + X3_PIX - 1) / X3_PIX));
    }
    const long ncob = (p.Cout + X3_CO - 1) / X3_CO;
    if (p.Cout <= 32) {
        r.kernel = 1; r.workgroups = r.tiles;
    } else if (svi_switches().vae_pair) {
        r.kernel = 2; r.workgroups = (r.tiles + 1) / 2 * ncob;
    } else {
        r.kernel = 3; r.workgroups = r.tiles * ncob;
    }
    return r;
}

svi_status launch_conv_planes(const ConvP& p, hipStream_t st) {
    SVI_REQUIRE(conv_planes_ok(p) && p.in_h && p.in_l, "conv: this layer cannot take fp16 input planes");
    SVI_REQUIRE(p.ld_out % 4 == 0 && (!p.res || p.ld_res % 4 == 0) && (((uintptr_t)p.res | (uintptr_t)p.out) & 15) == 0, "conv: output / residual alignment");
    const long pixels = (long)(p.To - p.t_begin) * p.Ho * p.Wo;
    if (pixels <= 0) return SVI_OK;
    const ConvPlanesPlan pl = conv_planes_plan(p);
    ConvP q = p;
    q.ord_T = pl.ord_T;
    if (pl.ord_T) { q.ord_Lf = pl.ord_Lf; q.ord_G = pl.ord_G; }
    SVI_REQUIRE(pl.workgroups < (1L << 31), "conv: too many workgroups");
    dim3 grid((unsigned)pl.workgroups, 1), block(512);
    if (pl.kernel == 1) {
        SVI_REQUIRE((p.Cout + 3) / 4 * 4 <= p.ld_out && (!p.res || (p.Cout + 3) / 4 * 4 <= p.ld_res), "conv: a narrow head writes whole groups of four channels (Cout=%d, ld_out=%d)", p.Cout, p.ld_out);
        SVI_REQUIRE(p.Cout % 4 != 0 || (((uintptr_t)p.bias | (uintptr_t)p.w2_inv) & 15) == 0, "conv: bias / scale alignment");
        SVI_TRY(svi_ensure_lds(reinterpret_cast<const void*>(conv_dma2h_kernel<1>), 2 * D2_STAGE));
        hipLaunchKernelGGL(conv_dma2h_kernel<1>, grid, block, 2 * D2_STAGE, st, q);
    } else {
        SVI_REQUIRE((((uintptr_t)p.bias) & 15) == 0, "conv: bias alignment");
        if (pl.kernel == 2) {
            SVI_TRY(svi_ensure_lds(reinterpret_cast<const void*>(conv_dma2h_pair_kernel), D2P_LDS));
            hipLaunchKernelGGL(conv_dma2h_pair_kernel, grid, block, D2P_LDS, st, q);
        } else {
            SVI_TRY(svi_ensure_lds(reinterpret_cast<const void*>(conv_dma2h_kernel<3>), 2 * D2_STAGE));
            hipLaunchKernelGGL(conv_dma2h_kernel<3>, grid, block, 2 * D2_STAGE, st, q);
        }
    }
    SVI_LAUNCH_CHECK();
    return SVI_OK;
}

bool conv_x3_ok(const ConvP& p) {
    const bool no_x3 = svi_switches().vae_exact_fp32 != 0;
    return p.w3 && !no_x3 && !p.act_silu && !p.out_bf16 && p.Cout >= 64 && p.Cout % 4 == 0 && p.ld_out % 4 == 0 && (!p.res || p.ld_res % 4 == 0) &&
           (p.out_mode == 0 || (p.Cout / 2) % 4 == 0) && (((uintptr_t)p.bias | (uintptr_t)p.res | (uintptr_t)p.out) & 15) == 0 &&
           p.kt * p.kh * p.kw <= 32 &&
           (long)(p.kt + 3) * p.Hi * p.Wi * p.ld_in * 4 < 0xFFFFF000L &&
           (long)3 * p.plane_w3 * 2 < 0xFFFFF000L;
}

svi_status launch_conv(const ConvP& p, hipStream_t st) {
    SVI_REQUIRE(p.Cin % 4 == 0 && p.ld_in % 4 == 0 && p.ld_w % 4 == 0, "conv: Cin/ld must be multiples of 4 (Cin=%d)", p.Cin);
    SVI_REQUIRE(!p.up_phase || (conv_x3_ok(p) && !p.ups && p.out_mode == 0), "conv: an upsample phase runs on the three-term kernel only");
    const long pixels = (long)(p.To - p.t_begin) * p.Ho * p.Wo;
    if (pixels <= 0) return SVI_OK;
    if (conv_x3_ok(p)) {
        dim3 grid3((unsigned)((pixels + X3_PIX - 1) / X3_PIX), (unsigned)((p.Cout + X3_CO - 1) / X3_CO)), block3(512);
        ConvP pa = p;
        if (p.w2h && p.w2_inv && p.in_scale > 0.f && !svi_switches().vae_no_x2h && (((uintptr_t)p.w2_inv) & 15) == 0 && p.Cin % 32 == 0 && !p.ups && !p.up_phase &&
            (long)(p.kt + 3) * p.Hi * p.Wi * p.ld_in * 4 < 0xFFE00000L && (long)2 * p.plane_w3 * 2 < 0xFFE00000L) {
            SVI_TRY(svi_ensure_lds(reinterpret_cast<const void*>(conv_igemm_x3_kernel<true>), 2 * X2H_STAGE));
            hipLaunchKernelGGL(conv_igemm_x3_kernel<true>, grid3, block3, 2 * X2H_STAGE, st, pa);
        } else {
            SVI_TRY(svi_ensure_lds(reinterpret_cast<const void*>(conv_igemm_x3_kernel<false>), 2 * X3_STAGE));
            hipLaunchKernelGGL(conv_igemm_x3_kernel<false>, grid3, block3, 2 * X3_STAGE, st, pa);
        }
        SVI_LAUNCH_CHECK();
        return SVI_OK;
    }
    const int NT = p.Cout > 32 ? 3 : 1;
    dim3 grid((unsigned)((pixels + 127) / 128), (unsigned)((p.Cout + 32 * NT - 1) / (32 * NT))), block(256);
    SVI_TRY(svi_ensure_lds(reinterpret_cast<const void*>(conv_igemm_kernel<3>), 2 * (128 * 128 + 3 * 32 * 128)));
    SVI_TRY(svi_ensure_lds(reinterpret_cast<const void*>(conv_igemm_kernel<1>), 2 * (128 * 128 + 1 * 32 * 128)));
    if (NT == 3)
        hipLaunchKernelGGL(conv_igemm_kernel<3>, grid, block, 2 * (128 * 128 + 3 * 32 * 128), st, p);
    else
        hipLaunchKernelGGL(conv_igemm_kernel<1>, grid, block, 2 * (128 * 128 + 1 * 32 * 128), st, p);
    SVI_LAUNCH_CHECK();
    return SVI_OK;
}

svi_status launch_conv_up_phases(ConvP p, const bf16* w3_up, hipStream_t st) {
    p.ups = 0; p.kh = p.kw = 2;
    p.Ho = p.Hi; p.Wo = p.Wi;
    p.plane_w3 = (long)p.kt * 4 * p.Cout * p.ld_w3;
    p.w2h = nullptr; p.w = nullptr;
    for (int ph = 0; ph < 4; ++ph) {
        p.up_phase = 1 + ph;
        p.ph = 1 - (ph >> 1); p.pw = 1 - (ph & 1);
        p.w3 = w3_up + (long)ph * 3 * p.plane_w3;
        SVI_TRY(launch_conv(p, st));
    }
    return SVI_OK;
}

}

svi_status svi_vae_conv_choose(int Cin, int Cout, int kt, int frames, int Ho, int Wo, int64_t* out8) {
    SVI_REQUIRE(out8 && Cin > 0 && Cout > 0 && kt > 0 && frames > 0 && Ho > 0 && Wo > 0, "svi_vae_conv_plan: bad argument");
    for (int i = 0; i < 8; ++i) out8[i] = 0;
    alignas(16) static const float dummy[4] = {0.f, 0.f, 0.f, 0.f};
    ConvP p{};
    p.Ti = p.To = frames; p.Hi = p.Ho = Ho; p.Wi = p.Wo = Wo; p.Cin = p.ld_in = Cin; p.Cout = Cout;
    p.kt = kt; p.kh = p.kw = 3; p.st = p.sh = p.sw = 1; p.pt = kt - 1; p.ph = p.pw = 1;
    p.ld_w3 = (Cin + 31) / 32 * 32; p.plane_w3 = (long)kt * 9 * Cout * p.ld_w3;
    p.w2h = dummy; p.w2_inv = dummy; p.in_scale = 1.f;
    if (!conv_planes_ok(p)) return SVI_OK;
    const ConvPlanesPlan pl = conv_planes_plan(p);
    const long HoWo = (long)Ho * Wo, P_total = (long)frames * HoWo, frame_bytes = HoWo * Cin * 2;
    const int per_wg = pl.kernel == 2 ? 2 : 1;
    long span = 0, desc_frames = 0;
    for (long w = 0; w * per_wg < pl.tiles; ++w) {
        int t0 = -1;
        for (int s = 0; s < per_wg && w * per_wg + s < pl.tiles; ++s) {
            const long p0 = conv_tile_at(pl.ord_T, pl.ord_Lf, pl.ord_G, w * per_wg + s) * X3_PIX;
            const int t_first = (int)(std::max(std::min(p0 - 1, P_total - 1), 0L) / HoWo);
            const int t_last = (int)(std::min(p0 - 2 + D2_ROWS, P_total - 1) / HoWo);
            const int base = std::max(t_first * p.st - p.pt, 0), top = std::min(t_last * p.st - p.pt + kt - 1, p.Ti - 1);
            desc_frames = std::max<long>(desc_frames, top - base + 1);
            const int t = (int)(p0 / HoWo);
            if (t0 >= 0) span = std::max<long>(span, t > t0 ? t - t0 : t0 - t);
            t0 = t;
        }
    }
    out8[0] = pl.kernel; out8[1] = pl.ord_T; out8[2] = pl.ord_Lf; out8[3] = pl.ord_G; out8[4] = pl.workgroups;
    out8[5] = span; out8[6] = desc_frames * frame_bytes; out8[7] = (long)(kt + 3) * frame_bytes;
    return SVI_OK;
}

svi_status svi_vae_tile_order_fill(int ord_T, int ord_Lf, int ord_G, int64_t* out) {
    SVI_REQUIRE(out && ord_T > 0 && ord_Lf > 0 && ord_G > 0 && ord_G <= ord_Lf, "svi_vae_tile_order: bad argument");
    for (long i = 0; i < (long)ord_T * ord_Lf; ++i) out[i] = conv_tile_at(ord_T, ord_Lf, ord_G, i);
    return SVI_OK;
}

svi_status svi_launch_gemm_f32(const float* A, int lda, const float* W, int ldw, const float* bias, float* Cm, int ldc, int M, int N, int K,
                               const float* res, int ldres, hipStream_t st) {
    SVI_REQUIRE(M >= 0 && N > 0 && K > 0 && K % 4 == 0 && lda % 4 == 0 && ldw % 4 == 0, "gemm_f32: K and the leading dimensions must be multiples of 4");
    SVI_REQUIRE(lda >= K && ldw >= K && ldc >= N && (!res || ldres >= N), "gemm_f32: leading dimensions too small");
    SVI_REQUIRE((((uintptr_t)A | (uintptr_t)W) & 15) == 0, "gemm_f32: operands must be 16-byte aligned");
    if (M == 0) return SVI_OK;
    ConvP g{};
    g.in = A; g.Ti = 1; g.Hi = 1; g.Wi = M; g.Cin = K; g.ld_in = lda;
    g.w = W; g.ld_w = ldw; g.bias = bias;
    g.out = Cm; g.To = 1; g.Ho = 1; g.Wo = M; g.Cout = N; g.ld_out = ldc;
    g.kt = g.kh = g.kw = 1; g.st = g.sh = g.sw = 1;
    g.res = res; g.ld_res = ldres;
    return launch_conv(g, st);
}

namespace {
__device__ __forceinline__ float norm_silu_el(float x, float factor, float g, int do_silu) {
    const float y = x * factor * g;
    if (!do_silu) return y;
    const float e = __builtin_amdgcn_exp2f(y * -1.4426950408889634f);
    return y * __builtin_amdgcn_rcpf(1.0f + e);
}
template <int MAXI>
__global__ __launch_bounds__(256) void rms_silu_kernel(const float* __restrict__ in, float* __restrict__ out, long pixels,
                                                       int C, const float* __restrict__ gamma, int do_silu) {
    const long px = (long)blockIdx.x * 32 + (threadIdx.x >> 3);
    const int q = threadIdx.x & 7;
    if (px >= pixels) return;
    const float* ip = in + px * C;
    f32x4 v[MAXI];
    float ss = 0.f;
#pragma unroll
    for (int i = 0; i < MAXI; ++i) {
        const int c = 4 * q + 32 * i;
        if (c < C) v[i] = *reinterpret_cast<const f32x4*>(ip + c);
        else v[i] = f32x4{0.f, 0.f, 0.f, 0.f};
        ss += v[i][0] * v[i][0];
        ss += v[i][1] * v[i][1];
        ss += v[i][2] * v[i][2];
        ss += v[i][3] * v[i][3];
    }
#pragma unroll
    for (int o = 4; o > 0; o >>= 1) ss += __shfl_xor(ss, o);
    const float factor = sqrtf((float)C) / fmaxf(sqrtf(ss), 1e-12f);
    float* op = out + px * C;
#pragma unroll
    for (int i = 0; i < MAXI; ++i) {
        const int c = 4 * q + 32 * i;
        if (c < C) {
            const float g[4] = {gamma[c], gamma[c + 1], gamma[c + 2], gamma[c + 3]};
            f32x4 y;
#pragma unroll
            for (int e = 0; e < 4; ++e) y[e] = norm_silu_el(v[i][e], factor, g[e], do_silu);
            *reinterpret_cast<f32x4*>(op + c) = y;
        }
    }
}

svi_status launch_rms_silu(const float* in, float* out, long pixels, int C, const float* gamma, int do_silu, hipStream_t st) {
    SVI_REQUIRE(C <= 384 && C % 4 == 0, "vae rms norm: C=%d (need a multiple of 4, at most 384)", C);
    SVI_REQUIRE(((uintptr_t)in % 16) == 0 && ((uintptr_t)out % 16) == 0, "vae rms norm: activations must be 16-byte aligned");
    if (pixels <= 0) return SVI_OK;
    dim3 grid((unsigned)((pixels + 31) / 32)), block(256);
    if (C <= 96) hipLaunchKernelGGL(rms_silu_kernel<3>, grid, block, 0, st, in, out, pixels, C, gamma, do_silu);
    else if (C <= 192) hipLaunchKernelGGL(rms_silu_kernel<6>, grid, block, 0, st, in, out, pixels, C, gamma, do_silu);
    else hipLaunchKernelGGL(rms_silu_kernel<12>, grid, block, 0, st, in, out, pixels, C, gamma, do_silu);
    SVI_LAUNCH_CHECK();
    return SVI_OK;
}

template <int MAXI>
__global__ __launch_bounds__(256) void rms_silu_planes_kernel(const float* __restrict__ in, unsigned short* __restrict__ out_h, unsigned short* __restrict__ out_l,
                                                              long pixels, int C, const float* __restrict__ gamma, int do_silu, float s) {
    const long px = (long)blockIdx.x * 32 + (threadIdx.x >> 3);
    const int q = threadIdx.x & 7;
    if (px >= pixels) return;
    const float* ip = in + px * C;
    f32x4 v[MAXI][2];
    float ss = 0.f;
#pragma unroll
    for (int i = 0; i < MAXI; ++i) {
        const int c = 8 * q + 64 * i;
#pragma unroll
        for (int hf = 0; hf < 2; ++hf) {
            if (c < C) v[i][hf] = *reinterpret_cast<const f32x4*>(ip + c + 4 * hf);
            else v[i][hf] = f32x4{0.f, 0.f, 0.f, 0.f};
            ss += v[i][hf][0] * v[i][hf][0];
            ss += v[i][hf][1] * v[i][hf][1];
            ss += v[i][hf][2] * v[i][hf][2];
            ss += v[i][hf][3] * v[i][hf][3];
        }
    }
#pragma unroll
    for (int o = 4; o > 0; o >>= 1) ss += __shfl_xor(ss, o);
    const float factor = sqrtf((float)C) / fmaxf(sqrtf(ss), 1e-12f);
#pragma unroll
    for (int i = 0; i < MAXI; ++i) {
        const int c = 8 * q + 64 * i;
        if (c < C) {
            u16x8 hh, ll;
#pragma unroll
            for (int e = 0; e < 8; ++e) {
                const float t = norm_silu_el(v[i][e >> 2][e & 3], factor, gamma[c + e], do_silu);
                const f16 hw = (f16)(t * s);
                hh[e] = bits16(hw);
                ll[e] = bits16((f16)__builtin_fmaf(t, s, -(float)hw));
            }
            *reinterpret_cast<u16x8*>(out_h + px * C + c) = hh;
            *reinterpret_cast<u16x8*>(out_l + px * C + c) = ll;
        }
    }
}

svi_status launch_rms_silu_planes(const float* in, unsigned short* out_h, unsigned short* out_l, long pixels, int C, const float* gamma, int do_silu, float s,
                                  hipStream_t st) {
    SVI_REQUIRE(C <= 384 && C % 8 == 0 && s > 0.f, "vae rms norm (planes): C=%d", C);
    SVI_REQUIRE(((uintptr_t)in % 16) == 0 && ((uintptr_t)out_h % 16) == 0 && ((uintptr_t)out_l % 16) == 0, "vae rms norm (planes): alignment");
    if (pixels <= 0) return SVI_OK;
    dim3 grid((unsigned)((pixels + 31) / 32)), block(256);
    if (C <= 128) hipLaunchKernelGGL(rms_silu_planes_kernel<2>, grid, block, 0, st, in, out_h, out_l, pixels, C, gamma, do_silu, s);
    else if (C <= 192) hipLaunchKernelGGL(rms_silu_planes_kernel<3>, grid, block, 0, st, in, out_h, out_l, pixels, C, gamma, do_silu, s);
    else hipLaunchKernelGGL(rms_silu_planes_kernel<6>, grid, block, 0, st, in, out_h, out_l, pixels, C, gamma, do_silu, s);
    SVI_LAUNCH_CHECK();
    return SVI_OK;
}

__global__ __launch_bounds__(256) void softmax_rows_kernel(float* __restrict__ s, int rows, int cols, int ld, float scale) {
    const int row = blockIdx.x * 4 + (threadIdx.x >> 6);
    const int lane = threadIdx.x & 63;
    if (row >= rows) return;
    float* r = s + (long)row * ld;
    float mx = -INFINITY;
    for (int c = lane; c < cols; c += 64) mx = fmaxf(mx, r[c]);
    mx = wave_max(mx);
    float sum = 0.f;
    for (int c = lane; c < cols; c += 64) {
        const float e = expf((r[c] - mx) * scale);
        r[c] = e;
        sum += e;
    }
    sum = wave_sum(sum);
    const float inv = 1.0f / sum;
    for (int c = lane; c < cols; c += 64) r[c] *= inv;
}

__global__ __launch_bounds__(256) void transpose_f32_kernel(const float* __restrict__ in, int ldi, float* __restrict__ out,
                                                            int ldo, int rows, int cols) {
    __shared__ float tile[64][65];
    const int r0 = blockIdx.y * 64, c0 = blockIdx.x * 64;
    const int tx = threadIdx.x & 63, ty = threadIdx.x >> 6;
    for (int i = ty; i < 64; i += 4) {
        const int r = r0 + i, c = c0 + tx;
        tile[i][tx] = (r < rows && c < cols) ? in[(long)r * ldi + c] : 0.f;
    }
    __syncthreads();
    for (int i = ty; i < 64; i += 4) {
        const int c = c0 + i, r = r0 + tx;
        if (c < cols && r < rows) out[(long)c * ldo + r] = tile[tx][i];
    }
}

__global__ void latent_in_kernel(const float* __restrict__ z, float* __restrict__ out, long thw, const float* __restrict__ mean,
                                 const float* __restrict__ inv_std) {
    const long i = (long)blockIdx.x * blockDim.x + threadIdx.x;
    if (i >= thw * 16) return;
    const int c = (int)(i & 15);
    const long sp = i >> 4;
    out[i] = z[(long)c * thw + sp] / inv_std[c] + mean[c];
}
__global__ void latent_out_kernel(const float* __restrict__ mu, int ld, float* __restrict__ z, long thw, const float* __restrict__ mean,
                                  const float* __restrict__ inv_std) {
    const long i = (long)blockIdx.x * blockDim.x + threadIdx.x;
    if (i >= thw * 16) return;
    const int c = (int)(i / thw);
    const long sp = i - (long)c * thw;
    z[i] = (mu[sp * ld + c] - mean[c]) * inv_std[c];
}
__global__ void video_in_kernel(const float* __restrict__ v, float* __restrict__ out, long thw) {
    const long i = (long)blockIdx.x * blockDim.x + threadIdx.x;
    if (i >= thw * 4) return;
    const int c = (int)(i & 3);
    out[i] = c < 3 ? v[(long)c * thw + (i >> 2)] : 0.f;
}
__global__ void video_out_kernel(const float* __restrict__ in, int ld, float* __restrict__ v, long thw) {
    const long i = (long)blockIdx.x * blockDim.x + threadIdx.x;
    if (i >= thw * 3) return;
    const int c = (int)(i / thw);
    const long sp = i - (long)c * thw;
    v[i] = fminf(fmaxf(in[sp * ld + c], -1.f), 1.f);
}
// ... 231 lines not shown
    add_res(h, e + "middle.0.", top, top); add_attn(h, e + "middle.1.", top); add_res(h, e + "middle.2.", top, top);
    add_gamma(h, e + "head.0.gamma", top, false);
    add_conv(h, e + "head.2", 2 * z, top, 3, 3, 3);
    add_conv(h, "model.conv1", 2 * z, 2 * z, 1, 1, 1);
    add_conv(h, "model.conv2", z, z, 1, 1, 1);
    int dd[5] = {base * mult[3], base * mult[3], base * mult[2], base * mult[1], base * mult[0]};
    add_conv(h, d + "conv1", dd[0], z, 3, 3, 3);
    add_res(h, d + "middle.0.", dd[0], dd[0]); add_attn(h, d + "middle.1.", dd[0]); add_res(h, d + "middle.2.", dd[0], dd[0]);
    const bool tup[3] = {true, true, false};
    idx = 0;
    for (int i = 0; i < 4; ++i) {
        int di = dd[i];
        const int dout = dd[i + 1];
        if (i >= 1) di = di / 2;
        for (int r = 0; r < 3; ++r) { add_res(h, d + "upsamples." + std::to_string(idx++) + ".", di, dout); di = dout; }
        if (i != 3) {
            const std::string p = d + "upsamples." + std::to_string(idx++) + ".";
            add_conv(h, p + "resample.1", dout / 2, dout, 1, 3, 3, true);
            h->convs[p + "resample.1"].upsample = true;
            if (tup[i]) add_conv(h, p + "time_conv", dout * 2, dout, 3, 1, 1);
        }
    }
    add_gamma(h, d + "head.0.gamma", dd[4], false);
    add_conv(h, d + "head.2", 3, dd[4], 3, 3, 3);
}

Tens alloc_t(svi_vae* h, int T, int H, int W, int C) {
    Tens t; t.T = T; t.H = H; t.W = W; t.C = C;
    if (h->dry) { if (t.elems() > h->dry_max) h->dry_max = t.elems(); t.p = nullptr; return t; }
    for (int i = 0; i < h->nslots; ++i)
        if (!h->slot_used[i]) { h->slot_used[i] = 1; t.p = reinterpret_cast<float*>(h->pool + (size_t)i * h->slot_bytes); return t; }
    t.p = nullptr;
    return t;
}
void free_t(svi_vae* h, Tens& t) {
    if (h->dry || !t.p) { t.p = nullptr; return; }
    const size_t i = (reinterpret_cast<char*>(t.p) - h->pool) / h->slot_bytes;
    h->slot_used[i] = 0;
    t.p = nullptr;
}
#define NEED(t) do { if (!h->dry && !(t).p) { svi_set_error("VAE tensor pool exhausted"); return SVI_ERR_OOM; } } while (0)

static svi_status grid_256(long n, const char* what, dim3* grid) {
    const long groups = (n + 255) / 256;
    SVI_REQUIRE(n >= 0 && groups < (1L << 31), "%s is too large for one launch (%ld elements)", what, n);
    *grid = dim3((unsigned)groups);
    return SVI_OK;
}

static float scale_of_bound(float bound) {
    if (!(bound > 0.f && bound < 1e30f)) return 0.f;
    int e = 0;
    (void)frexpf(bound, &e);
    return ldexpf(1.0f, 15 - e);
}

static ConvP conv_params(const ConvW& c, const Tens& in, int stride_t, bool causal_pad, int sh, int ups, int zero_frame0, bool down_pad, int* To_, int* Ho_, int* Wo_) {
    ConvP p{};
    p.Ti = in.T; p.Hi = in.H; p.Wi = in.W; p.Cin = (c.Cin + 3) / 4 * 4; p.ld_in = in.C;
    p.kt = c.kt; p.kh = c.kh; p.kw = c.kw; p.st = stride_t; p.sh = sh; p.sw = sh;
    p.pt = causal_pad ? c.kt - 1 : 0; p.ph = down_pad ? 0 : c.kh / 2; p.pw = down_pad ? 0 : c.kw / 2;
    p.ups = ups; p.zero_frame0 = zero_frame0;
    const int Hv = ups ? 2 * in.H : in.H, Wv = ups ? 2 * in.W : in.W;
    *To_ = causal_pad ? in.T : (in.T - c.kt) / stride_t + 1;
    *Ho_ = down_pad ? Hv / 2 : Hv; *Wo_ = down_pad ? Wv / 2 : Wv;
    p.w = c.packed; p.ld_w = c.ldw; p.bias = c.b_user;
    p.w3 = c.packed3; p.ld_w3 = c.ldw3; p.plane_w3 = (long)c.kt * c.kh * c.kw * c.Cout * c.ldw3;
    p.w2h = c.packed2h; p.w2_inv = c.w2_scale ? c.w2_scale + c.Cout : nullptr;
    p.in_scale = scale_of_bound(in.bound);
    p.To = *To_; p.Ho = *Ho_; p.Wo = *Wo_; p.Cout = c.Cout;
    return p;
}

static float planes_scale_for(svi_vae* h, const std::string& name, const std::string& gname, const Tens& x) {
    if (h->dry) return 0.f;
    auto gb = h->gamma_bound.find(gname);
    Tens like = x;
    like.bound = gb == h->gamma_bound.end() ? 0.f : gb->second;
    int To, Ho, Wo;
    ConvP p = conv_params(h->convs.at(name), like, 1, true, 1, 0, 0, false, &To, &Ho, &Wo);
    return conv_planes_ok(p) ? p.in_scale : 0.f;
}

svi_status conv_layer(svi_vae* h, const std::string& name, const Tens& in, Tens* out, hipStream_t st, int stride_t = 1,
                      bool causal_pad = true, int sh = 1, int ups = 0, int zero_frame0 = 0, const Tens* res = nullptr,
                      bool down_pad = false) {
    const ConvW& c = h->convs.at(name);
    int To, Ho, Wo;
    ConvP p = conv_params(c, in, stride_t, causal_pad, sh, ups, zero_frame0, down_pad, &To, &Ho, &Wo);
    *out = alloc_t(h, To, Ho, Wo, c.Cout < 4 ? 4 : c.Cout);
    NEED(*out);
    if (h->dry) return SVI_OK;
    p.in = in.p; p.out = out->p; p.ld_out = out->C;
    p.res = res ? res->p : nullptr; p.ld_res = res ? res->C : 0;
    SviProfScope _p(PROF_VAE_CONV, st);
    if (in.plane_scale > 0.f) {
        SVI_REQUIRE(in.plane_scale == p.in_scale, "conv %s: input planes carry scale %g, the layer expects %g", name.c_str(), in.plane_scale, p.in_scale);
        p.in = nullptr;
        p.in_h = reinterpret_cast<const unsigned short*>(in.p);
        p.in_l = p.in_h + in.elems();
        return launch_conv_planes(p, st);
    }
    if (ups && c.packed3_up && svi_switches().vae_up_phases && !res) {
        ConvP q = p;
        q.ups = 0; q.kh = q.kw = 2; q.Ho = q.Hi; q.Wo = q.Wi; q.plane_w3 = (long)q.kt * 4 * q.Cout * q.ld_w3;
        if (conv_x3_ok(q)) return launch_conv_up_phases(p, c.packed3_up, st);
    }
    return launch_conv(p, st);
}

svi_status norm_act(svi_vae* h, const std::string& gname, const Tens& in, Tens* out, int do_silu, hipStream_t st, float plane_scale = 0.f) {
    *out = alloc_t(h, in.T, in.H, in.W, in.C);
    NEED(*out);
    if (h->dry) return SVI_OK;
    {
        auto gb = h->gamma_bound.find(gname);
        out->bound = gb == h->gamma_bound.end() ? 0.f : gb->second;
    }
    SviProfScope _p(PROF_VAE_OTHER, st);
    if (plane_scale > 0.f) {
        out->plane_scale = plane_scale;
        unsigned short* ph = reinterpret_cast<unsigned short*>(out->p);
        return launch_rms_silu_planes(in.p, ph, ph + in.elems(), (long)in.T * in.H * in.W, in.C, h->gammas.at(gname), do_silu, plane_scale, st);
    }
    return launch_rms_silu(in.p, out->p, (long)in.T * in.H * in.W, in.C, h->gammas.at(gname), do_silu, st);
}

svi_status res_block(svi_vae* h, const std::string& p, Tens* x, hipStream_t st) {
    Tens n, hmid, out, skip;
    const bool has_sc = h->convs.count(p + "shortcut") > 0;
    if (has_sc) SVI_TRY(conv_layer(h, p + "shortcut", *x, &skip, st));
    SVI_TRY(norm_act(h, p + "residual.0.gamma", *x, &n, 1, st, planes_scale_for(h, p + "residual.2", p + "residual.0.gamma", *x)));
    SVI_TRY(conv_layer(h, p + "residual.2", n, &hmid, st));
    free_t(h, n);
    SVI_TRY(norm_act(h, p + "residual.3.gamma", hmid, &n, 1, st, planes_scale_for(h, p + "residual.6", p + "residual.3.gamma", hmid)));
    free_t(h, hmid);
    SVI_TRY(conv_layer(h, p + "residual.6", n, &out, st, 1, true, 1, 0, 0, has_sc ? &skip : x));
    free_t(h, n);
    if (has_sc) free_t(h, skip);
    free_t(h, *x);
    *x = out;
    return SVI_OK;
}

svi_status attn_block(svi_vae* h, const std::string& p, Tens* x, hipStream_t st) {
    Tens n, qkv, out;
    SVI_TRY(norm_act(h, p + "norm.gamma", *x, &n, 0, st));
    SVI_TRY(conv_layer(h, p + "to_qkv", n, &qkv, st));
    free_t(h, n);
    const int C = x->C, hw = x->H * x->W;
    const int ldp = (hw + 3) / 4 * 4;
    Tens att = alloc_t(h, x->T, x->H, x->W, C);
    NEED(att);
    if (!h->dry) {
        const size_t need = ((size_t)hw * ldp + (size_t)C * ldp) * 4;
        if (h->attn_bytes < need) {
            if (h->attn_scratch) SVI_CHECK_HIP(hipFree(h->attn_scratch));
            h->attn_scratch = nullptr; h->attn_bytes = 0;
            hipError_t e = hipMalloc((void**)&h->attn_scratch, need);
            if (e != hipSuccess) { svi_set_error("hipMalloc(%zu B VAE attention scratch) failed", need); return SVI_ERR_OOM; }
            h->attn_bytes = need;
        }
        if (ldp != hw) SVI_CHECK_HIP(hipMemsetAsync(h->attn_scratch, 0, need, st));
        float* S = h->attn_scratch;
        float* VT = S + (size_t)hw * ldp;
        SviProfScope _pp(PROF_VAE_OTHER, st);
        for (int t = 0; t < x->T; ++t) {
            const float* q = qkv.p + (long)t * hw * 3 * C;
            ConvP g{};
            g.in = q; g.Ti = 1; g.Hi = 1; g.Wi = hw; g.Cin = C; g.ld_in = 3 * C;
            g.w = q + C; g.ld_w = 3 * C; g.bias = nullptr;
            g.out = S; g.To = 1; g.Ho = 1; g.Wo = hw; g.Cout = hw; g.ld_out = ldp;
            g.kt = g.kh = g.kw = 1; g.st = g.sh = g.sw = 1;
            SVI_TRY(launch_conv(g, st));
            hipLaunchKernelGGL(softmax_rows_kernel, dim3((hw + 3) / 4), dim3(256), 0, st, S, hw, hw, ldp, 1.0f / sqrtf((float)C));
            hipLaunchKernelGGL(transpose_f32_kernel, dim3((C + 63) / 64, (hw + 63) / 64), dim3(256), 0, st, q + 2 * C, 3 * C, VT, ldp, hw, C);
            SVI_LAUNCH_CHECK();
            ConvP o{};
            o.in = S; o.Ti = 1; o.Hi = 1; o.Wi = hw; o.Cin = ldp; o.ld_in = ldp;
            o.w = VT; o.ld_w = ldp; o.bias = nullptr;
            o.out = att.p + (long)t * hw * C; o.To = 1; o.Ho = 1; o.Wo = hw; o.Cout = C; o.ld_out = C;
            o.kt = o.kh = o.kw = 1; o.st = o.sh = o.sw = 1;
            SVI_TRY(launch_conv(o, st));
        }
    }
    free_t(h, qkv);
    SVI_TRY(conv_layer(h, p + "proj", att, &out, st, 1, true, 1, 0, 0, x));
    free_t(h, att);
    free_t(h, *x);
    *x = out;
    return SVI_OK;
}

static ConvP time_conv_params(const ConvW& c, const Tens& x, const Tens& out) {
    ConvP q{};
    q.in = x.p; q.Ti = x.T; q.Hi = x.H; q.Wi = x.W; q.Cin = c.Cin; q.ld_in = x.C;
    q.w = c.packed; q.ld_w = c.ldw; q.bias = c.b_user;
    q.w3 = c.packed3; q.ld_w3 = c.ldw3; q.plane_w3 = (long)c.kt * c.kh * c.kw * c.Cout * c.ldw3;
    q.out = out.p; q.Ho = x.H; q.Wo = x.W; q.Cout = c.Cout; q.ld_out = out.C;
    q.kt = 3; q.kh = q.kw = 1; q.sh = q.sw = 1;
    return q;
}

svi_status upsample_block(svi_vae* h, const std::string& p, Tens* x, bool temporal, hipStream_t st) {
    if (temporal && x->T > 1) {
        Tens up = alloc_t(h, 1 + 2 * (x->T - 1), x->H, x->W, x->C);
        NEED(up);
        if (!h->dry) {
            ConvP q = time_conv_params(h->convs.at(p + "time_conv"), *x, up);
            q.To = x->T; q.st = 1; q.pt = 2;
            q.zero_frame0 = 1; q.t_begin = 1; q.out_mode = 1;
            { SviProfScope _p(PROF_VAE_CONV, st); SVI_TRY(launch_conv(q, st)); }
            SVI_CHECK_HIP(hipMemcpyAsync(up.p, x->p, (size_t)x->H * x->W * x->C * 4, hipMemcpyDeviceToDevice, st));
        }
        free_t(h, *x);
        *x = up;
    }
    Tens out;
// ... 503 lines not shown
    auto c = h->convs.find(layer);
    if (c == h->convs.end() || (leaf != "weight" && leaf != "bias")) { svi_set_error("unknown VAE parameter '%s'", name); return SVI_ERR_INVALID; }
    ConvW& cw = c->second;
    if (leaf == "bias") {
        if (!(rank == 1 && shape[0] == cw.Cout)) { svi_set_error("shape mismatch for '%s'", name); return SVI_ERR_INVALID; }
        cw.b_user = reinterpret_cast<const float*>(dev_ptr);
        return SVI_OK;
    }
    if (!shape_ok(cw.shape)) { svi_set_error("shape mismatch for '%s'", name); return SVI_ERR_INVALID; }
    cw.w_user = reinterpret_cast<const float*>(dev_ptr);
    const int taps = cw.kt * cw.kh * cw.kw;
    const size_t n = (size_t)taps * cw.Cout * cw.ldw;
    if (!cw.packed) {
        hipError_t e = hipMalloc((void**)&cw.packed, n * 4);
        if (e != hipSuccess) { svi_set_error("hipMalloc(packed VAE weight) failed: %s", hipGetErrorString(e)); return SVI_ERR_OOM; }
    }
    dim3 grid;
    SVI_TRY(grid_256((long)n, name, &grid));
    hipLaunchKernelGGL(pack_weight_kernel, grid, dim3(256), 0, 0, cw.w_user, cw.packed, cw.Cout, cw.Cin, taps, cw.ldw);
    const bool narrow_head = cw.Cout <= 32 && cw.kh == 3 && cw.kw == 3 && cw.Cin % 32 == 0;
    if (cw.Cout >= 64 || narrow_head) {
        cw.ldw3 = (cw.Cin + 31) / 32 * 32;
        const size_t n3 = (size_t)taps * cw.Cout * cw.ldw3;
        if (!cw.packed3) {
            hipError_t e3 = hipMalloc((void**)&cw.packed3, 3 * n3 * 2);
            if (e3 != hipSuccess) { svi_set_error("hipMalloc(split VAE weight) failed: %s", hipGetErrorString(e3)); return SVI_ERR_OOM; }
        }
        dim3 grid3;
        SVI_TRY(grid_256((long)n3, name, &grid3));
        hipLaunchKernelGGL(pack_weight_x3_kernel, grid3, dim3(256), 0, 0, cw.w_user, cw.packed3, cw.Cout, cw.Cin, taps, cw.ldw3);
        if (!cw.packed2h) {
            hipError_t e2 = hipMalloc((void**)&cw.packed2h, 2 * n3 * 2);
            if (e2 == hipSuccess) e2 = hipMalloc((void**)&cw.w2_scale, (size_t)2 * cw.Cout * 4);
            if (e2 != hipSuccess) { svi_set_error("hipMalloc(fp16 split VAE weight) failed: %s", hipGetErrorString(e2)); return SVI_ERR_OOM; }
        }
        if (cw.upsample && cw.kt == 1 && cw.kh == 3 && cw.kw == 3) {
            const size_t nu = (size_t)4 * 3 * 4 * cw.Cout * cw.ldw3;
            if (!cw.packed3_up) {
                hipError_t eu = hipMalloc((void**)&cw.packed3_up, nu * 2);
                if (eu != hipSuccess) { svi_set_error("hipMalloc(upsample phase weights) failed: %s", hipGetErrorString(eu)); return SVI_ERR_OOM; }
            }
            const size_t nt = (size_t)4 * 4 * cw.Cout * cw.ldw3;
            SVI_TRY(grid_256((long)nt, name, &grid));
            hipLaunchKernelGGL(pack_weight_up_x3_kernel, grid, dim3(256), 0, 0, cw.w_user, cw.packed3_up, cw.Cout, cw.Cin, cw.ldw3);
        }
        hipLaunchKernelGGL(weight_row_scale_kernel, dim3(cw.Cout), dim3(256), 0, 0, cw.w_user, cw.w2_scale, cw.w2_scale + cw.Cout, (long)cw.Cin * taps);
        hipLaunchKernelGGL(pack_weight_x2h_kernel, grid3, dim3(256), 0, 0, cw.w_user, cw.w2_scale, cw.packed2h, cw.Cout, cw.Cin, taps, cw.ldw3);
    }
    SVI_LAUNCH_CHECK();
    h->pack_pending = true;
    return SVI_OK;
}

extern "C" svi_status svi_vae_check_bound(svi_vae* h) {
    SVI_REQUIRE(h, "null handle");
    return check_bound(h);
}

static svi_status vae_prepare(svi_vae* h) {
    SVI_TRY(check_bound(h));
    if (h->pack_pending) {
        SVI_CHECK_HIP(hipStreamSynchronize(nullptr));
        h->pack_pending = false;
    }
    if (!h->consts) {
        float host[32];
        for (int i = 0; i < 16; ++i) { host[i] = kMean[i]; host[16 + i] = 1.0f / kStd[i]; }
        SVI_CHECK_HIP(hipMalloc((void**)&h->consts, sizeof(host)));
        SVI_CHECK_HIP(hipMemcpy(h->consts, host, sizeof(host), hipMemcpyHostToDevice));
        SVI_CHECK_HIP(hipDeviceSynchronize());
    }
    return SVI_OK;
}

extern "C" svi_status svi_vae_decode(svi_vae* h, const float* latents, float* video, int32_t T, int32_t hh, int32_t ww,
                                     svi_stream stream) {
    SVI_REQUIRE(h && latents && video && T > 0 && hh > 0 && ww > 0, "svi_vae_decode: bad argument");
    SVI_REQUIRE_DEVICE(h);
    SVI_TRY(vae_prepare(h));
    hipStream_t st = reinterpret_cast<hipStream_t>(stream);
    return sized_run(h, [&] { return decode_graph(h, latents, video, T, hh, ww, nullptr, 0, 0, st); });
}

extern "C" svi_status svi_vae_split_plan(int32_t hh, int32_t ww, int32_t parts_h, int32_t parts_w, int32_t part, int32_t* out24) {
    SVI_REQUIRE(out24, "svi_vae_split_plan: null argument");
    SplitPlan pl{};
    SVI_TRY(split_plan(hh, ww, parts_h, parts_w, part, &pl));
    plan_to_flat(pl, out24);
    return SVI_OK;
}

static svi_status decode_with_plan(svi_vae* h, const float* latents, float* video, int T, int hh, int ww, const SplitPlan& pl, int32_t video_ld_h, int32_t video_ld_w,
                                   hipStream_t st) {
    SVI_REQUIRE(video_ld_h >= 8 * (pl.own[1] - pl.own[0]) && video_ld_w >= 8 * (pl.own[3] - pl.own[2]),
                "svi_vae_decode_part: video pitches %d rows x %d elements are smaller than the owned window %d x %d", video_ld_h, video_ld_w,
                8 * (pl.own[1] - pl.own[0]), 8 * (pl.own[3] - pl.own[2]));
    SVI_TRY(vae_prepare(h));
    return sized_run(h, [&] { return decode_graph(h, latents, video, T, hh, ww, &pl, video_ld_h, video_ld_w, st); });
}

extern "C" svi_status svi_vae_decode_part(svi_vae* h, const float* latents, float* video, int32_t T, int32_t hh, int32_t ww, int32_t parts_h, int32_t parts_w,
                                          int32_t part, int32_t video_ld_h, int32_t video_ld_w, svi_stream stream) {
    SVI_REQUIRE(h && latents && video && T > 0 && hh > 0 && ww > 0, "svi_vae_decode_part: bad argument");
    SVI_REQUIRE_DEVICE(h);
    SplitPlan pl{};
    SVI_TRY(split_plan(hh, ww, parts_h, parts_w, part, &pl));
    if (parts_h * parts_w == 1 && video_ld_h == 8 * hh && video_ld_w == 8 * ww) return svi_vae_decode(h, latents, video, T, hh, ww, stream);
    return decode_with_plan(h, latents, video, T, hh, ww, pl, video_ld_h, video_ld_w, reinterpret_cast<hipStream_t>(stream));
}

extern "C" svi_status svi_vae_decode_planned(svi_vae* h, const float* latents, float* video, int32_t T, int32_t hh, int32_t ww, const int32_t* plan24,
                                             int32_t video_ld_h, int32_t video_ld_w, svi_stream stream) {
    SVI_REQUIRE(h && latents && video && plan24 && T > 0 && hh > 0 && ww > 0, "svi_vae_decode_planned: bad argument");
    SVI_REQUIRE_DEVICE(h);
    const SplitPlan pl = plan_from_flat<SplitPlan>(plan24);
    SVI_TRY(split_plan_check(pl, hh, ww));
    return decode_with_plan(h, latents, video, T, hh, ww, pl, video_ld_h, video_ld_w, reinterpret_cast<hipStream_t>(stream));
}

extern "C" svi_status svi_vae_encode(svi_vae* h, const float* video, float* latents, int32_t T, int32_t H, int32_t W,
                                     svi_stream stream) {
    SVI_REQUIRE(h && video && latents && T > 0 && H > 0 && W > 0, "svi_vae_encode: bad argument");
    SVI_REQUIRE_DEVICE(h);
    SVI_REQUIRE((T - 1) % 4 == 0 && H % 8 == 0 && W % 8 == 0, "svi_vae_encode: needs T = 1+4k frames and H, W multiples of 8 (got %d, %d, %d)", T, H, W);
    SVI_TRY(vae_prepare(h));
    hipStream_t st = reinterpret_cast<hipStream_t>(stream);
    return sized_run(h, [&] { return encode_graph(h, video, latents, T, H, W, st); });
}

extern "C" svi_status svi_vae_encode_split_plan(int32_t hh, int32_t ww, int32_t parts_h, int32_t parts_w, int32_t part, int32_t* out34) {
    SVI_REQUIRE(out34, "svi_vae_encode_split_plan: null argument");
    EncSplitPlan pl{};
    SVI_TRY(encode_split_plan(hh, ww, parts_h, parts_w, part, &pl));
    plan_to_flat(pl, out34);
    return SVI_OK;
}

static svi_status encode_with_plan(svi_vae* h, const float* video, float* feat_out, int T, int H, int W, const EncSplitPlan& pl, int32_t ld_h, int32_t ld_w, hipStream_t st) {
    SVI_REQUIRE(ld_h >= pl.own[1] - pl.own[0] && ld_w >= pl.own[3] - pl.own[2], "svi_vae_encode_part: feature pitches %d rows x %d pixels are smaller than the owned window %d x %d",
                ld_h, ld_w, pl.own[1] - pl.own[0], pl.own[3] - pl.own[2]);
    SVI_REQUIRE(reinterpret_cast<uintptr_t>(feat_out) % 16 == 0, "svi_vae_encode_part: feat_out must be 16-byte aligned");
    SVI_TRY(vae_prepare(h));
    return sized_run(h, [&] { return encode_part_graph(h, video, feat_out, T, H, W, pl, ld_h, ld_w, st); });
}

extern "C" svi_status svi_vae_encode_part(svi_vae* h, const float* video, float* feat_out, int32_t T, int32_t H, int32_t W, int32_t parts_h, int32_t parts_w,
                                          int32_t part, int32_t ld_h, int32_t ld_w, svi_stream stream) {
    SVI_REQUIRE(h && video && feat_out && T > 0 && H > 0 && W > 0, "svi_vae_encode_part: bad argument");
    SVI_REQUIRE_DEVICE(h);
    SVI_REQUIRE((T - 1) % 4 == 0 && H % 8 == 0 && W % 8 == 0, "svi_vae_encode_part: needs T = 1+4k frames and H, W multiples of 8 (got %d, %d, %d)", T, H, W);
    EncSplitPlan pl{};
    SVI_TRY(encode_split_plan(H / 8, W / 8, parts_h, parts_w, part, &pl));
    return encode_with_plan(h, video, feat_out, T, H, W, pl, ld_h, ld_w, reinterpret_cast<hipStream_t>(stream));
}

extern "C" svi_status svi_vae_encode_planned(svi_vae* h, const float* video, float* feat_out, int32_t T, int32_t H, int32_t W, const int32_t* plan34,
                                             int32_t ld_h, int32_t ld_w, svi_stream stream) {
    SVI_REQUIRE(h && video && feat_out && plan34 && T > 0 && H > 0 && W > 0, "svi_vae_encode_planned: bad argument");
    SVI_REQUIRE_DEVICE(h);
    SVI_REQUIRE((T - 1) % 4 == 0 && H % 8 == 0 && W % 8 == 0, "svi_vae_encode_planned: needs T = 1+4k frames and H, W multiples of 8 (got %d, %d, %d)", T, H, W);
    const EncSplitPlan pl = plan_from_flat<EncSplitPlan>(plan34);
    SVI_TRY(encode_split_plan_check(pl, H / 8, W / 8));
    return encode_with_plan(h, video, feat_out, T, H, W, pl, ld_h, ld_w, reinterpret_cast<hipStream_t>(stream));
}

extern "C" svi_status svi_vae_encode_tail(svi_vae* h, const float* feat, float* latents, int32_t Tl, int32_t hh, int32_t ww, svi_stream stream) {
// ... 237 lines not shown
```

stable-video-infinity_amd/svi_hip/_lib.py:

```python
from __future__ import annotations

import ctypes as C
import os

_HERE = os.path.dirname(os.path.abspath(__file__))
LIB_PATH = os.environ.get("SVI_HIP_LIB") or os.path.join(_HERE, "libsvi_hip.so")

SVI_OK = 0
SVI_BF16, SVI_F32, SVI_F16, SVI_E4M3 = 0, 1, 2, 3
EPI_BIAS, EPI_BIAS_GELU_TANH, EPI_BIAS_GATE_RES, EPI_BIAS_GELU_ERF, EPI_BIAS_SILU, EPI_BIAS_RELU = 0, 1, 2, 3, 4, 5

_vp, _i32, _i64, _f32 = C.c_void_p, C.c_int32, C.c_int64, C.c_float


class DitConfig(C.Structure):
    _fields_ = [("dim", _i32), ("in_dim", _i32), ("ffn_dim", _i32), ("out_dim", _i32), ("text_dim", _i32),
                ("freq_dim", _i32), ("eps", _f32), ("patch_t", _i32), ("patch_h", _i32), ("patch_w", _i32),
                ("num_heads", _i32), ("num_layers", _i32), ("has_image_input", _i32), ("enable_multitalk", _i32)]


class T5Config(C.Structure):
    _fields_ = [("vocab", _i32), ("dim", _i32), ("dim_attn", _i32), ("dim_ffn", _i32), ("num_heads", _i32), ("num_layers", _i32),
                ("num_buckets", _i32), ("max_dist", _i32), ("shared_pos", _i32)]


class ClipConfig(C.Structure):
    _fields_ = [("image_size", _i32), ("patch_size", _i32), ("dim", _i32), ("mlp_ratio", _i32), ("num_heads", _i32), ("num_layers", _i32),
                ("layers_used", _i32), ("norm_eps", _f32)]


class W2vConfig(C.Structure):
    _fields_ = [("conv_dim", _i32), ("hidden", _i32), ("ffn", _i32), ("num_heads", _i32), ("num_layers", _i32), ("pos_kernel", _i32),
                ("pos_groups", _i32), ("eps", _f32)]


SYMBOLS = [
    ("svi_last_error", C.c_char_p, []),
    ("svi_abi_version", _i32, []),
    ("svi_device_count", _i32, []),
    ("svi_switches_reload", _i32, []),
    ("svi_switch_state", _i32, [C.c_char_p]),
    ("svi_dit_create", _i32, [C.POINTER(DitConfig), C.POINTER(_vp)]),
    ("svi_dit_destroy", _i32, [_vp]),
    ("svi_dit_bind_weight", _i32, [_vp, C.c_char_p, _vp, _i32, C.POINTER(_i64), _i32]),
    ("svi_dit_check_bound", _i32, [_vp]),
    ("svi_dit_forward", _i32, [_vp, _vp, _vp, _vp, _vp, _vp, _vp, _vp, _i32, _i32, _i32, _i32, _i32, _vp]),
    ("svi_dit_sp_begin", _i32, [_vp, _vp, _vp, _vp, _vp, _vp, _vp, _i32, _i32, _i32, _i32, _i32, _i32, _vp]),
    ("svi_dit_sp_begin_pair", _i32, [_vp, _vp, _vp, _vp, _vp, _vp, _vp, _vp, _i32, _i32, _i32, _i32, _i32, _i32, _vp]),
    ("svi_dit_sp_block_qkv", _i32, [_vp, _i32, _vp, _vp, _vp, _i32, _i32, _i32, _vp]),
    ("svi_dit_sp_block_qkv_part", _i32, [_vp, _i32, _vp, _vp, _vp, _i32, _i32, _i32, _i32, _vp]),
    ("svi_sp_unpack_vt", _i32, [_vp, _vp, _i32, _i32, _i32, _i32, _i32, _i32, _i32, _vp]),
    ("svi_sp_unpack_out", _i32, [_vp, _vp, _i32, _i32, _i32, _i32, _i32, _vp]),
    ("svi_dit_sp_block_rest", _i32, [_vp, _i32, _vp, _vp]),
    ("svi_dit_sp_tea", _i32, [_vp, _i32, _vp, _vp]),
    ("svi_dit_sp_head", _i32, [_vp, _vp, _vp]),
    ("svi_dit_unpatchify", _i32, [_vp, _vp, _vp, _i32, _i32, _i32, _vp]),
    ("svi_dit_head_ld", _i32, [_vp]),
    ("svi_dit_generation", _i64, [_vp]),
    ("svi_stream_buffers_release", _i32, [_vp, _i32]),
    ("svi_attention_last_flagged", _i32, [_vp, C.POINTER(_i32), C.POINTER(_i32)]),
    ("svi_attention_vt_fwd", _i32, [_vp, _i32, _vp, _i32, _vp, _i32, _vp, _i32, _i32, _i32, _i32, _i32, _vp]),
    ("svi_attention_frames_fwd", _i32, [_vp, _i32, _vp, _i32, _vp, _i32, _vp, _i32, _i32, _i32, _i32, _i32, _i32, _vp]),
    ("svi_dit_set_audio", _i32, [_vp, _vp, _vp, _i32]),
    ("svi_dit_audio_slot", _i32, [_vp, _i32, _vp, _vp, _i32, _vp]),
    ("svi_dit_forward_talk3", _i32, [_vp, _vp, _vp, _vp, _vp, _vp, _vp, _vp, _vp, _vp, _vp, _i32, _i32, _i32, _i32, _vp]),
    ("svi_dit_forward_talk3_tea", _i32, [_vp, _vp, _vp, _vp, _vp, _vp, _vp, _vp, _vp, _vp, _vp, _i32, _i32, _i32, _i32, _i32, _i32, _i32, _vp, _vp, _vp, _vp]),
    ("svi_audio_windows", _i32, [_vp, _i32, _i32, _i32, _i32, _i32, _vp, _vp, _vp]),
    ("svi_dit_audio_slot_windows", _i32, [_vp, _i32, _vp, _i32, _i32, _i32, _i32, _vp]),
    ("svi_cfg3_step", _i32, [_vp, _vp, _vp, _vp, _i64, _f32, _f32, _f32, _vp]),
    ("svi_dit_time_mod", _i32, [_vp, _vp, _vp, _i32, _vp]),
    ("svi_dit_forward_tea", _i32, [_vp, _vp, _vp, _vp, _vp, _vp, _vp, _vp, _i32, _i32, _i32, _i32, _i32, _i32, _vp, _vp]),
    ("svi_dit_forward_cfg_pair", _i32, [_vp, _vp, _vp, _vp, _vp, _vp, _vp, _vp, _vp, _vp, _i32, _i32, _i32, _i32, _i32, _vp]),
    ("svi_dit_forward_cfg_pair_tea", _i32, [_vp, _vp, _vp, _vp, _vp, _vp, _vp, _vp, _vp, _vp, _i32, _i32, _i32, _i32, _i32, _i32, _vp, _vp, _vp]),
    ("svi_dit_context_cache", _i32, [_vp, _i32]),
    ("svi_dit_context_refill", _i32, [_vp, _vp, _vp, _i32, _vp]),
    ("svi_linear_row_stats", _i32, [_vp, _i32, _vp, _i32, _vp, _i32, _i32, _i32, _i32, _vp, _f32, _vp, _i32, _vp, _vp]),
    ("svi_cross_attention_fwd", _i32, [_vp, _i32, _vp, _i32, _vp, _i32, _vp, _i32, _i32, _i32, _i32, _vp, _vp, _vp, _f32, _vp]),
    ("svi_dit_block_forward", _i32, [_vp, _i32, _vp, _vp, _vp, _i32, _i32, _i32, _i32, _vp]),
    ("svi_attention_fwd", _i32, [_vp, _vp, _vp, _vp, _i32, _i32, _i32, _i32, _i32, _vp]),
    ("svi_layernorm_modulate", _i32, [_vp, _vp, _i32, _i32, _f32, _vp, _vp, _vp, _vp, _vp]),
    ("svi_rmsnorm_rope", _i32, [_vp, _i32, _i32, _i32, _vp, _f32, _i32, _i32, _i32, _i32, _i32, _vp]),
    ("svi_rmsnorm_rope_qk", _i32, [_vp, _i32, _i32, _i32, _vp, _vp, _f32, _f32, _f32, _i32, _i32, _i32, _i32, _i32, _i32, _vp]),
    ("svi_gemm_bf16", _i32, [_vp, _i32, _vp, _i32, _vp, _i32, _i32, _i32, _i32, _vp, _i32, _i32, _vp, _vp, _i32, _vp]),
    ("svi_gemm_bf16_pair", _i32, [_vp, _i32, _vp, _i32, _vp, _i32, _i32, _i32, _i32, _vp, _i32, _i32, _vp, _vp, _i32, _vp, _vp, _i32, _i32, _i32, _vp]),
    ("svi_gemm_bf16_w8", _i32, [_vp, _i32, _vp, _i32, _vp, _i32, _i32, _i32, _i32, _vp, _i32, _i32, _vp, _vp, _i32, _vp, _vp, _i32, _i32, _i32, _vp]),
    ("svi_cfg_step", _i32, [_vp, _vp, _vp, _i64, _f32, _f32, _vp]),
    ("svi_mx8_quantize", _i32, [_vp, _i32, _i32, _i32, _vp, _i32, _vp, _i32, _vp]),
    ("svi_gemm_mx8", _i32, [_vp, _i32, _vp, _i32, _vp, _i32, _vp, _i32, _i32, _i32, _i32, _vp, _i32, _vp, _vp, _i32, _vp]),
    ("svi_dit_bind_ffn_fp8", _i32, [_vp, _i32, _i32, _vp]),
    ("svi_dit_ffn_mx8", _i32, [_vp, _i32]),
    ("svi_gemm_mx8_wscaled", _i32, [_vp, _i32, _vp, _i32, _vp, _i32, _vp, _i32, _i32, _i32, _i32, _vp, _i32, _vp]),
    ("svi_dit_proj_mx8", _i32, [_vp, _i32]),
    ("svi_fp8_e4m3_to_bf16", _i32, [_vp, _vp, _i64, _vp]),
    ("svi_f32_to_fp8_e4m3", _i32, [_vp, _i32, _vp, _i64, _vp]),
    ("svi_lora_merge_e4m3", _i32, [_vp, _i32, _i32, _vp, _vp, _i32, _i32, _f32, _vp]),
    ("svi_gemm_bf16_skinny", _i32, [_vp, _i32, _vp, _i32, _vp, _i32, _i32, _i32, _i32, _vp, _i32, _vp, _vp, _i32, _i32, _vp]),
    ("svi_gemm_plan", _i32, [_i32, _i32, _i32, _i32, _i32, _i32, C.POINTER(_i32)]),
    ("svi_gemm_w8_plan", _i32, [_i32, _i32, _i32, _i32, _i32, _i32, C.POINTER(_i32)]),
    ("svi_attention_plan", _i32, [_i32, _i32, _i32, _i32, C.POINTER(_i32)]),
    ("svi_vae_conv_plan", _i32, [_i32, _i32, _i32, _i32, _i32, _i32, C.POINTER(_i64)]),
    ("svi_vae_tile_order", _i32, [_i32, _i32, _i32, C.POINTER(_i64)]),
    ("svi_prof_enable", _i32, [_i32]),
    ("svi_prof_summary", _i32, [C.c_char_p, _i64]),
    ("svi_prof_select", _i32, [C.c_char_p]),
    ("svi_vae_create", _i32, [C.POINTER(_vp)]),
    ("svi_vae_destroy", _i32, [_vp]),
    ("svi_vae_bind_weight", _i32, [_vp, C.c_char_p, _vp, _i32, C.POINTER(_i64), _i32]),
    ("svi_vae_check_bound", _i32, [_vp]),
    ("svi_video_to_u8", _i32, [_vp, _vp, _i32, _i32, _i32, _vp]),
    ("svi_u8_to_video", _i32, [_vp, _vp, _i32, _i32, _i32, _vp]),
    ("svi_vae_decode", _i32, [_vp, _vp, _vp, _i32, _i32, _i32, _vp]),
    ("svi_vae_encode", _i32, [_vp, _vp, _vp, _i32, _i32, _i32, _vp]),
    ("svi_vae_tiled_decode", _i32, [_vp, _vp, _vp, _i32, _i32, _i32, _i32, _i32, _i32, _i32, _vp]),
    ("svi_vae_tiled_encode", _i32, [_vp, _vp, _vp, _i32, _i32, _i32, _i32, _i32, _i32, _i32, _vp]),
    ("svi_vae_split_plan", _i32, [_i32, _i32, _i32, _i32, _i32, C.POINTER(_i32)]),
    ("svi_vae_decode_part", _i32, [_vp, _vp, _vp, _i32, _i32, _i32, _i32, _i32, _i32, _i32, _i32, _vp]),
    ("svi_vae_decode_planned", _i32, [_vp, _vp, _vp, _i32, _i32, _i32, C.POINTER(_i32), _i32, _i32, _vp]),
    ("svi_vae_encode_split_plan", _i32, [_i32, _i32, _i32, _i32, _i32, C.POINTER(_i32)]),
    ("svi_vae_encode_part", _i32, [_vp, _vp, _vp, _i32, _i32, _i32, _i32, _i32, _i32, _i32, _i32, _vp]),
    ("svi_vae_encode_planned", _i32, [_vp, _vp, _vp, _i32, _i32, _i32, C.POINTER(_i32), _i32, _i32, _vp]),
    ("svi_vae_encode_tail", _i32, [_vp, _vp, _vp, _i32, _i32, _i32, _vp]),
    ("svi_pose_create", _i32, [_i32, _i32, C.POINTER(_vp)]),
    ("svi_pose_destroy", _i32, [_vp]),
    ("svi_pose_bind_weight", _i32, [_vp, C.c_char_p, _vp, _i32, C.POINTER(_i64), _i32]),
    ("svi_pose_check_bound", _i32, [_vp]),
    ("svi_pose_tokens", _i32, [_vp, _i32, _i32, _i32, C.POINTER(_i32), C.POINTER(_i32), C.POINTER(_i32)]),
    ("svi_pose_forward", _i32, [_vp, _vp, _vp, _i32, _i32, _i32, _vp]),
    ("svi_pose_window", _i32, [_vp, _vp, _i32, _i32, _i32, _i32, _i32, _i32, _i32, _i32, _vp]),
    ("svi_pose_window_plan", _i32, [_i32, _i32, _i32, _i32, _i32, _i32, _i32, _i32, C.POINTER(_i32), C.POINTER(_i32), C.POINTER(_i32)]),
    ("svi_t5_create", _i32, [C.POINTER(T5Config), C.POINTER(_vp)]),
    ("svi_t5_destroy", _i32, [_vp]),
    ("svi_t5_bind_weight", _i32, [_vp, C.c_char_p, _vp, _i32, C.POINTER(_i64), _i32]),
    ("svi_t5_check_bound", _i32, [_vp]),
    ("svi_t5_forward", _i32, [_vp, _vp, _i32, _i32, _i32, _vp, _vp]),
    ("svi_t5_relative_buckets", _i32, [_i32, _i32, _i32, C.POINTER(_i32)]),
    ("svi_t5_device_buckets", _i32, [_vp, _i32, C.POINTER(_i32)]),
    ("svi_clip_create", _i32, [C.POINTER(ClipConfig), C.POINTER(_vp)]),
    ("svi_clip_destroy", _i32, [_vp]),
    ("svi_clip_bind_weight", _i32, [_vp, C.c_char_p, _vp, _i32, C.POINTER(_i64), _i32]),
    ("svi_clip_check_bound", _i32, [_vp]),
    ("svi_clip_tokens", _i32, [_vp, C.POINTER(_i32), C.POINTER(_i32)]),
    ("svi_clip_encode_image", _i32, [_vp, _vp, _i32, _i32, _i32, _vp, _vp]),
    ("svi_w2v_create", _i32, [C.POINTER(W2vConfig), C.POINTER(_vp)]),
    ("svi_w2v_destroy", _i32, [_vp]),
    ("svi_w2v_bind_weight", _i32, [_vp, C.c_char_p, _vp, _i32, C.POINTER(_i64), _i32]),
    ("svi_w2v_check_bound", _i32, [_vp]),
    ("svi_w2v_frames", _i32, [_i64, C.POINTER(_i64)]),
    ("svi_w2v_forward", _i32, [_vp, _vp, _i64, _i32, _vp, _i32, _vp]),
    ("svi_w2v_forward_stage", _i32, [_vp, _vp, _i64, _i32, _i32, _vp, _i64, _vp]),
    ("svi_w2v_set_max_frames", _i32, [_vp, _i32]),
    ("svi_encoder_attention_f32", _i32, [_vp, _i32, _vp, _i32, _vp, _i32, _vp, _i32, _i32, _i32, _i32, _i32, _f32, _i32, _vp]),
]

_lib = None


def lib() -> C.CDLL:
    global _lib
    if _lib is None:
        if not os.path.exists(LIB_PATH):
            raise RuntimeError(
                f"{LIB_PATH} is missing: build it with `python __graft_entry__.py build` "
                "(hipcc --offload-arch=gfx950).  svi_hip has no CPU or PyTorch fallback.")
        l = C.CDLL(LIB_PATH)
        for name, res, args in SYMBOLS:
            fn = getattr(l, name)
            fn.restype, fn.argtypes = res, args
        _lib = l
    return _lib


def last_error() -> str:
    return (lib().svi_last_error() or b"").decode("utf-8", "replace")


def check(status: int, what: str = "") -> None:
    if status != SVI_OK:
        raise RuntimeError(f"svi_hip{': ' + what if what else ''} failed (status {status}): {last_error()}")


def ptr(t) -> int:
    return None if t is None else t.data_ptr()


def current_stream() -> int:
    import torch
    return torch.cuda.current_stream().cuda_stream


_switch_epoch = 0


def switch_epoch() -> int:
    return _switch_epoch


def set_switch(name: str, value=None) -> None:
    global _switch_epoch
    _switch_epoch += 1
    if value is None:
        os.environ.pop(name, None)
    else:
        os.environ[name] = str(value)
    check(lib().svi_switches_reload(), "svi_switches_reload")


def release_stream_buffers(stream=None) -> None:
    check(lib().svi_stream_buffers_release(_vp(stream.cuda_stream) if stream is not None else None, 1 if stream is None else 0), "svi_stream_buffers_release")


def prof_enable(on: bool) -> None:
    check(lib().svi_prof_enable(1 if on else 0), "svi_prof_enable")


def gemm_plan(M: int, N: int, K: int, epilogue: int = 0, skinny: bool = False, compute_units: int = 256) -> int:
    out = _i32(0)
    check(lib().svi_gemm_plan(M, N, K, epilogue, 1 if skinny else 0, compute_units, C.byref(out)), "svi_gemm_plan")
    return out.value


def attention_plan(s_q: int, s_kv: int, heads: int, compute_units: int = 256) -> dict:
    out = (_i32 * 4)()
    check(lib().svi_attention_plan(s_q, s_kv, heads, compute_units, out), "svi_attention_plan")
    return {"kernel": out[0], "whole": out[1], "pieces": out[2], "workgroups": out[3]}


VAE_CONV_KERNELS = {0: None, 1: "dma2h<1>", 3: "dma2h<3>", 2: "pair"}


def vae_conv_plan(Cin: int, Cout: int, kt: int, frames: int, Ho: int, Wo: int) -> dict:
    out = (_i64 * 8)()
    check(lib().svi_vae_conv_plan(Cin, Cout, kt, frames, Ho, Wo, out), "svi_vae_conv_plan")
    return {"kernel": VAE_CONV_KERNELS[out[0]], "ord_T": out[1], "ord_Lf": out[2], "ord_G": out[3], "workgroups": out[4], "pair_span": out[5],
            "desc_bytes": out[6], "guard_bytes": out[7]}


def vae_tile_order(ord_T: int, ord_Lf: int, ord_G: int) -> list:
    out = (_i64 * (ord_T * ord_Lf))()
    check(lib().svi_vae_tile_order(ord_T, ord_Lf, ord_G, out), "svi_vae_tile_order")
    return list(out)


def pose_window_plan(N: int, h: int, w: int, H: int, W: int, F: int, m: int, k: int) -> dict:
    frame, row, col = (_i32 * max(F, 1))(), (_i32 * max(H, 1))(), (_i32 * max(W, 1))()
    check(lib().svi_pose_window_plan(N, h, w, H, W, F, m, k, frame, row, col), "svi_pose_window_plan")
    return {"frame_src": list(frame), "row_src": list(row), "col_src": list(col)}


def vae_split_plan(hh: int, ww: int, parts_h: int, parts_w: int, part: int) -> dict:
    out = (_i32 * 24)()
    check(lib().svi_vae_split_plan(hh, ww, parts_h, parts_w, part, out), "svi_vae_split_plan")
    return {"owned": tuple(out[0:4]), "halo": tuple(out[4:8]), "padded": [tuple(out[8 + 4 * s:12 + 4 * s]) for s in range(4)]}


VAE_ENCODE_ENTRIES = ("video", "stage0", "stage1", "stage2", "stage3")


def vae_encode_split_plan(hh: int, ww: int, parts_h: int, parts_w: int, part: int) -> dict:
    out = (_i32 * 34)()
    check(lib().svi_vae_encode_split_plan(hh, ww, parts_h, parts_w, part, out), "svi_vae_encode_split_plan")
    return {"owned": tuple(out[0:4]), "reach": [tuple(out[4 + 2 * k:6 + 2 * k]) for k in range(5)], "rects": [tuple(out[14 + 4 * k:18 + 4 * k]) for k in range(5)]}


def prof_select(tags=None) -> None:
    arg = None if not tags else ",".join(tags).encode()
    check(lib().svi_prof_select(arg), "svi_prof_select")


def prof_summary() -> dict:
    import json
    buf = C.create_string_buffer(8192)
    check(lib().svi_prof_summary(buf, len(buf)), "svi_prof_summary")
    return json.loads(buf.value.decode())
```

stable-video-infinity_amd/svi_hip/vae.py:

```python
from __future__ import annotations

import ctypes as C
import math
from typing import Dict, List, Optional, Sequence

import torch

from . import _lib as L


def vae_param_shapes() -> Dict[str, tuple]:
    s: Dict[str, tuple] = {}

    def conv3(n, o, i, k=(3, 3, 3)):
        s[n + ".weight"] = (o, i, *k); s[n + ".bias"] = (o,)

    def conv2(n, o, i, k=3):
        s[n + ".weight"] = (o, i, k, k); s[n + ".bias"] = (o,)

    def res(p, i, o):
        s[p + "residual.0.gamma"] = (i, 1, 1, 1); conv3(p + "residual.2", o, i)
        s[p + "residual.3.gamma"] = (o, 1, 1, 1); conv3(p + "residual.6", o, o)
        if i != o:
            conv3(p + "shortcut", o, i, (1, 1, 1))
# ... 42 lines not shown
    for name, shape in vae_param_shapes().items():
        leaf = name.rsplit(".", 1)[-1]
        if leaf == "gamma":
            t = 1.0 + 0.1 * torch.randn(shape, generator=g, device=device)
        elif leaf == "weight":
            fan_in = 1
            for d in shape[1:]:
                fan_in *= d
            t = (torch.rand(shape, generator=g, device=device) * 2 - 1) / math.sqrt(fan_in)
        else:
            t = (torch.rand(shape, generator=g, device=device) * 2 - 1) * 0.05
        out[name] = t.float().contiguous()
    return out


def encoder_feature_channels() -> int:
    return vae_param_shapes()["model.encoder.middle.0.residual.2.weight"][1]


def default_vae_split(world: int) -> tuple:
    return {2: (1, 2), 4: (2, 2), 8: (2, 4)}.get(int(world), (1, int(world)))


def _encode_split_setting(vae_encode_split, group) -> dict:
    if vae_encode_split is None or vae_encode_split is False:
        return {}
    if vae_encode_split is True:
        if group is None:
            raise ValueError("vae_encode_split=True takes its grid from a process group (vae_group or a latency mode); name a grid (parts_h, parts_w) to split locally")
        import torch.distributed as dist
        vae_encode_split = default_vae_split(dist.get_world_size(group))
    split = (int(vae_encode_split[0]), int(vae_encode_split[1]))
    return dict(split=split, group=None if split == (1, 1) else group)


def latency_group(loop):
    import torch.distributed as dist
    if getattr(loop, "cfg_pair", None) is not None:
        return loop.cfg_pair.group if loop.cfg_pair.group is not None else dist.group.WORLD
    if getattr(loop, "sequence_parallel", False):
        return loop.sp_group if loop.sp_group is not None else dist.group.WORLD
    return None


class WanVideoVAE:
    upsampling_factor = 8

    def __init__(self):
        h = C.c_void_p()
        L.check(L.lib().svi_vae_create(C.byref(h)), "svi_vae_create")
        self._h = h
        self._params: Dict[str, torch.Tensor] = {}

    @classmethod
    def from_state_dict(cls, state_dict: Dict[str, torch.Tensor], device="cuda") -> "WanVideoVAE":
        v = cls()
        v.bind({k: t.to(device=device, dtype=torch.float32).contiguous() for k, t in state_dict.items()})
        return v

    @classmethod
    def from_module(cls, ref_vae) -> "WanVideoVAE":
        v = cls()
        v.bind({k: t.to(device="cuda", dtype=torch.float32).contiguous() for k, t in ref_vae.state_dict().items()})
        return v

    def bind(self, state_dict: Dict[str, torch.Tensor]) -> None:
        lib = L.lib()
        for name, t in state_dict.items():
            if not t.is_cuda or t.dtype != torch.float32 or not t.is_contiguous():
                raise RuntimeError(f"VAE parameter {name} must be a contiguous CUDA fp32 tensor")
            shape = (C.c_int64 * t.dim())(*t.shape)
            L.check(lib.svi_vae_bind_weight(self._h, name.encode(), t.data_ptr(), L.SVI_F32, shape, t.dim()), f"bind {name}")
            self._params[name] = t
        L.check(lib.svi_vae_check_bound(self._h), "svi_vae_check_bound")

    def __del__(self):
        try:
            if getattr(self, "_h", None):
                L.lib().svi_vae_destroy(self._h)
                self._h = None
        except Exception:
            pass

    def single_decode(self, hidden_state: torch.Tensor, device=None) -> torch.Tensor:
        z = hidden_state.to(device="cuda", dtype=torch.float32).contiguous()
        _, c, t, h, w = z.shape
        if c != 16:
            raise ValueError("latents must have 16 channels")
        out = torch.empty((1, 3, 1 + 4 * (t - 1), 8 * h, 8 * w), dtype=torch.float32, device=z.device)
        L.check(L.lib().svi_vae_decode(self._h, L.ptr(z), L.ptr(out), t, h, w, L.current_stream()), "svi_vae_decode")
        return out

    def single_encode(self, video: torch.Tensor, device=None) -> torch.Tensor:
        v = video.to(device="cuda", dtype=torch.float32).contiguous()
        _, c, t, h, w = v.shape
        if c != 3:
            raise ValueError("video must have 3 channels")
        out = torch.empty((1, 16, 1 + (t - 1) // 4, h // 8, w // 8), dtype=torch.float32, device=v.device)
        L.check(L.lib().svi_vae_encode(self._h, L.ptr(v), L.ptr(out), t, h, w, L.current_stream()), "svi_vae_encode")
        return out

    def tiled_decode(self, hidden_states: torch.Tensor, device, tile_size, tile_stride) -> torch.Tensor:
        z = hidden_states.to(device="cuda", dtype=torch.float32).contiguous()
        _, c, t, h, w = z.shape
        if c != 16:
            raise ValueError("latents must have 16 channels")
        out = torch.empty((1, 3, 4 * t - 3, 8 * h, 8 * w), dtype=torch.float32, device=z.device)
        L.check(L.lib().svi_vae_tiled_decode(self._h, L.ptr(z), L.ptr(out), t, h, w, int(tile_size[0]), int(tile_size[1]),
                                             int(tile_stride[0]), int(tile_stride[1]), L.current_stream()), "svi_vae_tiled_decode")
        return out

    def tiled_encode(self, video: torch.Tensor, device, tile_size, tile_stride) -> torch.Tensor:
        v = video.to(device="cuda", dtype=torch.float32).contiguous()
        _, c, t, h, w = v.shape
        if c != 3:
            raise ValueError("video must have 3 channels")
        out = torch.empty((1, 16, (t + 3) // 4, h // 8, w // 8), dtype=torch.float32, device=v.device)
        L.check(L.lib().svi_vae_tiled_encode(self._h, L.ptr(v), L.ptr(out), t, h, w, int(tile_size[0]), int(tile_size[1]),
                                             int(tile_stride[0]), int(tile_stride[1]), L.current_stream()), "svi_vae_tiled_encode")
        return out

    def encode(self, videos: Sequence[torch.Tensor], device=None, tiled=False, tile_size=(34, 34), tile_stride=(18, 16), split=None, group=None):
        if split is not None and tiled:
            raise ValueError("VAE encode: tiled=True blends overlapping tiles, split=(ph, pw) is the exact rank split; ask for one of them")
        if split is None and group is not None:
            raise ValueError("VAE encode: a group needs split=(parts_h, parts_w)")
        outs: List[torch.Tensor] = []
        for video in videos:
            video = video.unsqueeze(0)
            if split is not None:
                hs = self.split_encode(video, split, group)
            elif tiled:
                tile_size = (tile_size[0] * 8, tile_size[1] * 8)
                tile_stride = (tile_stride[0] * 8, tile_stride[1] * 8)
                hs = self.tiled_encode(video, device, tile_size, tile_stride)
            else:
                hs = self.single_encode(video, device)
            outs.append(hs.squeeze(0))
        return torch.stack(outs)

    def decode_part(self, hidden_state: torch.Tensor, split, part: int, out: Optional[torch.Tensor] = None, _short_halo: int = 0) -> torch.Tensor:
        z = hidden_state.to(device="cuda", dtype=torch.float32)
        z = (z[0] if z.dim() == 5 else z).contiguous()
        c, t, h, w = z.shape
        if c != 16:
            raise ValueError("latents must have 16 channels")
        ph, pw = int(split[0]), int(split[1])
        plan = L.vae_split_plan(h, w, ph, pw, int(part))
        h0, h1, w0, w1 = plan["owned"]
        oh, ow, tv = 8 * (h1 - h0), 8 * (w1 - w0), 1 + 4 * (t - 1)
        if out is None:
            out = torch.empty((3, tv, oh, ow), dtype=torch.float32, device=z.device)
        if not (out.is_cuda and out.dtype == torch.float32 and out.is_contiguous() and out.dim() == 4 and out.shape[0] == 3 and out.shape[1] == tv
                and out.shape[2] >= oh and out.shape[3] >= ow):
            raise ValueError(f"decode_part: out must be a contiguous CUDA fp32 [3, {tv}, >= {oh}, >= {ow}] tensor, got {tuple(out.shape)}")
        ld_h, ld_w = out.shape[2], out.shape[3]
        full = (ld_h, ld_w) == (8 * h, 8 * w)
        dst = out.data_ptr() + 4 * ((8 * h0) * ld_w + 8 * w0) if full else out.data_ptr()
        if _short_halo:
            s0 = plan["padded"][0]
            own = plan["owned"]
            cut = [min(s0[0] + _short_halo, own[0]), max(s0[1] - _short_halo, own[1]), min(s0[2] + _short_halo, own[2]), max(s0[3] - _short_halo, own[3])]
            flat = list(own) + list(plan["halo"]) + cut + [v for r in plan["padded"][1:] for v in r]
            L.check(L.lib().svi_vae_decode_planned(self._h, L.ptr(z), dst, t, h, w, (C.c_int32 * 24)(*flat), ld_h, ld_w, L.current_stream()), "svi_vae_decode_planned")
        else:
            L.check(L.lib().svi_vae_decode_part(self._h, L.ptr(z), dst, t, h, w, ph, pw, int(part), ld_h, ld_w, L.current_stream()), "svi_vae_decode_part")
# ... 129 lines not shown
```

Baseline: 1.015.

## Fuse RMS_norm+SiLU into VAE conv epilogue for 96-channel residual blocks

Adds an epilogue to the fp16-plane VAE convolution kernels that computes the per-pixel RMS norm, gain and SiLU across all 96 output channels inside the workgroup. It writes the split fp16 hi/lo planes that the next convolution reads directly. This removes a separate rms_silu launch and an fp32 round trip through memory for the middle activation of residual blocks. The fusion applies only when Cout equals the tile width. It adds cross-lane shuffles and a second epilogue variant, plus a test entry point for single residual blocks.

```diff
diff --git a/include/svi_hip.h b/include/svi_hip.h
--- a/include/svi_hip.h
+++ b/include/svi_hip.h
@@ -138,6 +138,9 @@
 svi_status svi_attention_plan(int32_t s_q, int32_t s_kv, int32_t heads, int32_t compute_units, int32_t* out4);
 svi_status svi_vae_conv_plan(int32_t Cin, int32_t Cout, int32_t kt, int32_t frames, int32_t Ho, int32_t Wo, int64_t* out8);
 svi_status svi_vae_tile_order(int32_t ord_T, int32_t ord_Lf, int32_t ord_G, int64_t* out);
+svi_status svi_vae_norm_fuse_plan(int32_t Cin, int32_t Cout, int32_t kt, int32_t consumer_planes, int32_t* fused);
+svi_status svi_vae_res_block(svi_vae* h, const char* prefix, const float* x, float* out, int32_t T, int32_t H, int32_t W,
+                             uint16_t* mid_h, uint16_t* mid_l, float* mid_f32, svi_stream stream);
 
 svi_status svi_layernorm_modulate(const void* x, void* out, int32_t rows, int32_t dim, float eps,
                                   const void* w, const void* b, const void* shift, const void* scale,
diff --git a/stable-video-infinity_amd/csrc/svi_api.hip b/stable-video-infinity_amd/csrc/svi_api.hip
--- a/stable-video-infinity_amd/csrc/svi_api.hip
+++ b/stable-video-infinity_amd/csrc/svi_api.hip
@@ -51,6 +51,7 @@
     s.vae_up_phases = env_int("SVI_VAE_UP_PHASES", 0, 1);
     s.vae_tile_order = env_int("SVI_VAE_TILE_ORDER", 0, 1);
     s.vae_pair = env_int("SVI_VAE_PAIR", 0, 1);
+    s.vae_fuse_norm = env_int("SVI_VAE_FUSE_NORM", 0, 1);
     s.mx8_fused = env_int("SVI_MX8_FUSED", 0, 1);
     s.qk_fused = env_int("SVI_QK_FUSED", 0, 1);
     s.attn_qk8 = env_int("SVI_ATTN_QK8", 0, 0) != 0;
@@ -556,6 +557,9 @@
 extern "C" svi_status svi_vae_tile_order(int32_t ord_T, int32_t ord_Lf, int32_t ord_G, int64_t* out) {
     return svi_vae_tile_order_fill(ord_T, ord_Lf, ord_G, out);
 }
+extern "C" svi_status svi_vae_norm_fuse_plan(int32_t Cin, int32_t Cout, int32_t kt, int32_t consumer_planes, int32_t* fused) {
+    return svi_vae_norm_fuse_choose(Cin, Cout, kt, consumer_planes, fused);
+}
 
 extern "C" svi_status svi_mx8_quantize(const void* x, int32_t ldx, int32_t rows, int32_t K, void* q, int32_t ldq, void* scales, int32_t sc_rows,
                                        svi_stream stream) {
diff --git a/stable-video-infinity_amd/csrc/svi_common.h b/stable-video-infinity_amd/csrc/svi_common.h
--- a/stable-video-infinity_amd/csrc/svi_common.h
+++ b/stable-video-infinity_amd/csrc/svi_common.h
@@ -61,6 +61,7 @@
     int vae_no_x2h = 0;
     int vae_dma = 1;
     int vae_pair = 1;
+    int vae_fuse_norm = 1;
     int vae_tile_order = 1;
     int vae_up_phases = 1;
     int flash_two_pass = 1;
@@ -180,6 +181,7 @@
 SviFlashSplit svi_flash_plan(int Lq, int Lk, int heads, int cus, int* kernel_out);
 svi_status svi_vae_conv_choose(int Cin, int Cout, int kt, int frames, int Ho, int Wo, int64_t* out8);
 svi_status svi_vae_tile_order_fill(int ord_T, int ord_Lf, int ord_G, int64_t* out);
+svi_status svi_vae_norm_fuse_choose(int Cin, int Cout, int kt, int consumer_planes, int32_t* fused);
 svi_status svi_launch_mx8_quantize(const bf16* x, int ldx, int rows, int K, unsigned char* q, int ldq, unsigned* scales, int sc_rows, hipStream_t st);
 svi_status svi_launch_gemm_mx8(const SviGemmArgs& g, const unsigned* a_scales, int sc_rows, hipStream_t st);
 svi_status svi_launch_gemm_mx8_wscaled(const SviGemmArgs& g, const unsigned* w_scales, int sc_rows, hipStream_t st);
diff --git a/stable-video-infinity_amd/csrc/svi_vae.hip b/stable-video-infinity_amd/csrc/svi_vae.hip
--- a/stable-video-infinity_amd/csrc/svi_vae.hip
+++ b/stable-video-infinity_amd/csrc/svi_vae.hip
@@ -31,6 +31,8 @@
     const unsigned short* in_h; const unsigned short* in_l;
     int ord_T, ord_Lf, ord_G;
     int up_phase;
+    unsigned short* out_h; unsigned short* out_l;
+    const float* nrm_gamma; float nrm_scale; int nrm_silu;
 };
 
 __device__ __forceinline__ int tile_off(int row, int chunk) { return row * 128 + ((chunk ^ ((row >> 1) & 7)) << 4); }
@@ -563,8 +565,85 @@
 }
 #define D2_A_PLANE (D2_ROWS * 64)
 #define D2_STAGE (2 * D2_A_PLANE + 6 * X3_W_PLANE)
-template <int NB>
+
+__device__ __forceinline__ float norm_silu_el(float x, float factor, float g, int do_silu) {
+    const float y = x * factor * g;
+    if (!do_silu) return y;
+    const float e = __builtin_amdgcn_exp2f(y * -1.4426950408889634f);
+    return y * __builtin_amdgcn_rcpf(1.0f + e);
+}
+__device__ __forceinline__ float rms_ss8(float ss, const f32x4& a, const f32x4& b) {
+    ss += a[0] * a[0]; ss += a[1] * a[1]; ss += a[2] * a[2]; ss += a[3] * a[3];
+    ss += b[0] * b[0]; ss += b[1] * b[1]; ss += b[2] * b[2]; ss += b[3] * b[3];
+    return ss;
+}
+__device__ __forceinline__ float rms_factor(float ss, int C) { return sqrtf((float)C) / fmaxf(sqrtf(ss), 1e-12f); }
+__device__ __forceinline__ void norm_silu_split8(const f32x4& a, const f32x4& b, float factor, const float* __restrict__ g, int do_silu, float s,
+                                                 u16x8* hh, u16x8* ll) {
+#pragma unroll
+    for (int e = 0; e < 8; ++e) {
+        const float t = norm_silu_el(e < 4 ? a[e & 3] : b[e & 3], factor, g[e], do_silu);
+        const f16 hw = (f16)(t * s);
+        (*hh)[e] = bits16(hw);
+        const unsigned short lw = bits16((f16)__builtin_fmaf(t, s, -(float)hw));
+        (*ll)[e] = (lw & 0x7fffu) ? lw : (unsigned short)0;
+    }
+}
+
+__device__ __forceinline__ void conv_norm_planes_epilogue(const ConvP& p, const f32x16 (&acc)[3], long po, bool live, int hi) {
+    const f32x4 zero4 = {0.f, 0.f, 0.f, 0.f};
+    const float inv_a = 1.0f / p.in_scale;
+    f32x4 a[3][2], b[3][2];
+#pragma unroll
+    for (int n = 0; n < 3; ++n)
+#pragma unroll
+        for (int m = 0; m < 2; ++m) {
+            f32x4 v[2];
+#pragma unroll
+            for (int r = 0; r < 2; ++r) {
+                const int rg = 2 * m + r;
+                const int co = 32 * n + 8 * rg + 4 * hi;
+                const f32x4 bv = p.bias ? *reinterpret_cast<const f32x4*>(p.bias + co) : zero4;
+                const f32x4 rv = (p.res && live) ? *reinterpret_cast<const f32x4*>(p.res + po * p.ld_res + co) : zero4;
+                const f32x4 sv = *reinterpret_cast<const f32x4*>(p.w2_inv + co) * inv_a;
+#pragma unroll
+                for (int e = 0; e < 4; ++e) v[r][e] = (acc[n][4 * rg + e] * sv[e] + bv[e]) + rv[e];
+                if (p.out && live) *reinterpret_cast<f32x4*>(p.out + po * p.ld_out + co) = v[r];
+            }
+#pragma unroll
+            for (int e = 0; e < 4; ++e) {
+                const float got = __shfl_xor(hi ? v[0][e] : v[1][e], 32);
+                a[n][m][e] = hi ? got : v[0][e];
+                b[n][m][e] = hi ? v[1][e] : got;
+            }
+        }
+    float t[2];
+#pragma unroll
+    for (int m = 0; m < 2; ++m) {
+        const float s_lo = rms_ss8(rms_ss8(0.f, a[0][m], b[0][m]), a[2][m], b[2][m]);
+        const float s_hi = rms_ss8(rms_ss8(0.f, a[1][m], b[1][m]), zero4, zero4);
+        t[m] = s_lo + s_hi;
+    }
+    float ss = t[0] + t[1];
+    ss += __shfl_xor(ss, 32);
+    const float factor = rms_factor(ss, p.Cout);
+#pragma unroll
+    for (int n = 0; n < 3; ++n)
+#pragma unroll
+        for (int m = 0; m < 2; ++m) {
+            const int c = 32 * n + 8 * (2 * m + hi);
+            u16x8 hh, ll;
+            norm_silu_split8(a[n][m], b[n][m], factor, p.nrm_gamma + c, p.nrm_silu, p.nrm_scale, &hh, &ll);
+            if (live) {
+                *reinterpret_cast<u16x8*>(p.out_h + po * p.Cout + c) = hh;
+                *reinterpret_cast<u16x8*>(p.out_l + po * p.Cout + c) = ll;
+            }
+        }
+}
+
+template <int NB, bool NORM = false>
 __global__ __launch_bounds__(512, 2) void conv_dma2h_kernel(ConvP p) {
+    static_assert(!NORM || NB == 3, "the fused RMS_norm epilogue needs the 96-channel tile");
 #ifdef SVI_D2_DENSE
     p.ld_in = 32; p.ld_w3 = 32;
 #endif
@@ -714,6 +793,10 @@
     }
 
     const long pp = p0 + 32 * wave + l31;
+    if constexpr (NORM) {
+        conv_norm_planes_epilogue(p, acc, pp + (long)p.t_out_off * HoWo, pp < P_total, hi);
+        return;
+    }
     if (pp >= P_total) return;
     const f32x4 zero4 = {0.f, 0.f, 0.f, 0.f};
     f32x4 bv[4 * NB], rv[4 * NB], sv[4 * NB];
@@ -764,6 +847,7 @@
 
 #define D2P_W_STAGE (6 * X3_W_PLANE)
 #define D2P_LDS (2 * D2P_W_STAGE + 2 * 2 * D2_A_PLANE)
+template <bool NORM>
 __global__ __launch_bounds__(512, 2) void conv_dma2h_pair_kernel(ConvP p) {
     constexpr int NB = 3, WP = 2 * NB;
     constexpr int A_SLOTS = 5, W_SLOTS = 5;
@@ -957,8 +1041,12 @@
 #pragma unroll
     for (int s = 0; s < 2; ++s) {
         const long pp = p0[s] + 32 * wave + l31;
+        const long po = pp + (long)p.t_out_off * HoWo;
+        if constexpr (NORM) {
+            conv_norm_planes_epilogue(p, acc[s], po, pp < P_total, hi);
+            continue;
+        }
         if (pp >= P_total) continue;
-        const long po = pp + (long)p.t_out_off * HoWo;
         long pq0 = 0;
         if (p.out_mode != 0) {
             const int t = (int)(pp / HoWo);
@@ -1022,8 +1110,19 @@
     return r;
 }
 
+bool conv_norm_fusable(const ConvP& p, float consumer_scale) {
+    return svi_switches().vae_fuse_norm && consumer_scale > 0.f && p.out_mode == 0 && p.Cout == X3_CO && conv_planes_ok(p);
+}
+
 svi_status launch_conv_planes(const ConvP& p, hipStream_t st) {
     SVI_REQUIRE(conv_planes_ok(p) && p.in_h && p.in_l, "conv: this layer cannot take fp16 input planes");
+    const bool norm = p.out_mode == 2;
+    if (norm) {
+        SVI_REQUIRE(p.Cout == X3_CO, "conv: the fused RMS_norm epilogue needs all output channels of a pixel in one workgroup (Cout = %d; this layer has %d and "
+                    "takes the two-launch path)", X3_CO, p.Cout);
+        SVI_REQUIRE(p.out_h && p.out_l && p.nrm_gamma && p.nrm_scale > 0.f && (((uintptr_t)p.out_h | (uintptr_t)p.out_l) & 15) == 0 && (!p.out || p.ld_out >= p.Cout),
+                    "conv: the fused RMS_norm epilogue needs its planes, gain vector and scale");
+    }
     SVI_REQUIRE(p.ld_out % 4 == 0 && (!p.res || p.ld_res % 4 == 0) && (((uintptr_t)p.res | (uintptr_t)p.out) & 15) == 0, "conv: output / residual alignment");
     const long pixels = (long)(p.To - p.t_begin) * p.Ho * p.Wo;
     if (pixels <= 0) return SVI_OK;
@@ -1040,9 +1139,15 @@
         hipLaunchKernelGGL(conv_dma2h_kernel<1>, grid, block, 2 * D2_STAGE, st, q);
     } else {
         SVI_REQUIRE((((uintptr_t)p.bias) & 15) == 0, "conv: bias alignment");
-        if (pl.kernel == 2) {
-            SVI_TRY(svi_ensure_lds(reinterpret_cast<const void*>(conv_dma2h_pair_kernel), D2P_LDS));
-            hipLaunchKernelGGL(conv_dma2h_pair_kernel, grid, block, D2P_LDS, st, q);
+        if (pl.kernel == 2 && norm) {
+            SVI_TRY(svi_ensure_lds(reinterpret_cast<const void*>(conv_dma2h_pair_kernel<true>), D2P_LDS));
+            hipLaunchKernelGGL(conv_dma2h_pair_kernel<true>, grid, block, D2P_LDS, st, q);
+        } else if (pl.kernel == 2) {
+            SVI_TRY(svi_ensure_lds(reinterpret_cast<const void*>(conv_dma2h_pair_kernel<false>), D2P_LDS));
+            hipLaunchKernelGGL(conv_dma2h_pair_kernel<false>, grid, block, D2P_LDS, st, q);
+        } else if (norm) {
+            SVI_TRY(svi_ensure_lds(reinterpret_cast<const void*>((conv_dma2h_kernel<3, true>)), 2 * D2_STAGE));
+            hipLaunchKernelGGL((conv_dma2h_kernel<3, true>), grid, block, 2 * D2_STAGE, st, q);
         } else {
             SVI_TRY(svi_ensure_lds(reinterpret_cast<const void*>(conv_dma2h_kernel<3>), 2 * D2_STAGE));
             hipLaunchKernelGGL(conv_dma2h_kernel<3>, grid, block, 2 * D2_STAGE, st, q);
@@ -1140,6 +1245,18 @@
     return SVI_OK;
 }
 
+svi_status svi_vae_norm_fuse_choose(int Cin, int Cout, int kt, int consumer_planes, int32_t* fused) {
+    SVI_REQUIRE(fused && Cin > 0 && Cout > 0 && kt > 0, "svi_vae_norm_fuse_plan: bad argument");
+    alignas(16) static const float dummy[4] = {0.f, 0.f, 0.f, 0.f};
+    ConvP p{};
+    p.Ti = p.To = 1; p.Hi = p.Ho = 16; p.Wi = p.Wo = 16; p.Cin = p.ld_in = Cin; p.Cout = Cout;
+    p.kt = kt; p.kh = p.kw = 3; p.st = p.sh = p.sw = 1; p.pt = kt - 1; p.ph = p.pw = 1;
+    p.ld_w3 = (Cin + 31) / 32 * 32; p.plane_w3 = (long)kt * 9 * Cout * p.ld_w3;
+    p.w2h = dummy; p.w2_inv = dummy; p.in_scale = 1.f;
+    *fused = conv_norm_fusable(p, consumer_planes ? 1.f : 0.f) ? 1 : 0;
+    return SVI_OK;
+}
+
 svi_status svi_vae_tile_order_fill(int ord_T, int ord_Lf, int ord_G, int64_t* out) {
     SVI_REQUIRE(out && ord_T > 0 && ord_Lf > 0 && ord_G > 0 && ord_G <= ord_Lf, "svi_vae_tile_order: bad argument");
     for (long i = 0; i < (long)ord_T * ord_Lf; ++i) out[i] = conv_tile_at(ord_T, ord_Lf, ord_G, i);
@@ -1162,12 +1279,6 @@
 }
 
 namespace {
-__device__ __forceinline__ float norm_silu_el(float x, float factor, float g, int do_silu) {
-    const float y = x * factor * g;
-    if (!do_silu) return y;
-    const float e = __builtin_amdgcn_exp2f(y * -1.4426950408889634f);
-    return y * __builtin_amdgcn_rcpf(1.0f + e);
-}
 template <int MAXI>
 __global__ __launch_bounds__(256) void rms_silu_kernel(const float* __restrict__ in, float* __restrict__ out, long pixels,
                                                        int C, const float* __restrict__ gamma, int do_silu) {
@@ -1232,27 +1343,18 @@
         for (int hf = 0; hf < 2; ++hf) {
             if (c < C) v[i][hf] = *reinterpret_cast<const f32x4*>(ip + c + 4 * hf);
             else v[i][hf] = f32x4{0.f, 0.f, 0.f, 0.f};
-            ss += v[i][hf][0] * v[i][hf][0];
-            ss += v[i][hf][1] * v[i][hf][1];
-            ss += v[i][hf][2] * v[i][hf][2];
-            ss += v[i][hf][3] * v[i][hf][3];
-        }
+        }
+        ss = rms_ss8(ss, v[i][0], v[i][1]);
     }
 #pragma unroll
     for (int o = 4; o > 0; o >>= 1) ss += __shfl_xor(ss, o);
-    const float factor = sqrtf((float)C) / fmaxf(sqrtf(ss), 1e-12f);
+    const float factor = rms_factor(ss, C);
 #pragma unroll
     for (int i = 0; i < MAXI; ++i) {
         const int c = 8 * q + 64 * i;
         if (c < C) {
             u16x8 hh, ll;
-#pragma unroll
-            for (int e = 0; e < 8; ++e) {
-                const float t = norm_silu_el(v[i][e >> 2][e & 3], factor, gamma[c + e], do_silu);
-                const f16 hw = (f16)(t * s);
-                hh[e] = bits16(hw);
-                ll[e] = bits16((f16)__builtin_fmaf(t, s, -(float)hw));
-            }
+            norm_silu_split8(v[i][0], v[i][1], factor, gamma + c, do_silu, s, &hh, &ll);
             *reinterpret_cast<u16x8*>(out_h + px * C + c) = hh;
             *reinterpret_cast<u16x8*>(out_l + px * C + c) = ll;
         }
@@ -1650,18 +1752,35 @@
     return conv_planes_ok(p) ? p.in_scale : 0.f;
 }
 
+struct NormFuse { std::string gname; int do_silu; float scale; Tens* f32; };
+
 svi_status conv_layer(svi_vae* h, const std::string& name, const Tens& in, Tens* out, hipStream_t st, int stride_t = 1,
                       bool causal_pad = true, int sh = 1, int ups = 0, int zero_frame0 = 0, const Tens* res = nullptr,
-                      bool down_pad = false) {
+                      bool down_pad = false, const NormFuse* nf = nullptr) {
     const ConvW& c = h->convs.at(name);
     int To, Ho, Wo;
     ConvP p = conv_params(c, in, stride_t, causal_pad, sh, ups, zero_frame0, down_pad, &To, &Ho, &Wo);
     *out = alloc_t(h, To, Ho, Wo, c.Cout < 4 ? 4 : c.Cout);
     NEED(*out);
+    if (nf && nf->f32) {
+        *nf->f32 = alloc_t(h, To, Ho, Wo, c.Cout);
+        NEED(*nf->f32);
+    }
     if (h->dry) return SVI_OK;
     p.in = in.p; p.out = out->p; p.ld_out = out->C;
     p.res = res ? res->p : nullptr; p.ld_res = res ? res->C : 0;
     SviProfScope _p(PROF_VAE_CONV, st);
+    if (nf) {
+        SVI_REQUIRE(in.plane_scale > 0.f && conv_norm_fusable(p, nf->scale), "conv %s: this layer cannot take the RMS_norm behind it into its epilogue", name.c_str());
+        auto gb = h->gamma_bound.find(nf->gname);
+        out->bound = gb == h->gamma_bound.end() ? 0.f : gb->second;
+        out->plane_scale = nf->scale;
+        p.out_mode = 2;
+        p.out_h = reinterpret_cast<unsigned short*>(out->p);
+        p.out_l = p.out_h + out->elems();
+        p.out = nf->f32 ? nf->f32->p : nullptr;
+        p.nrm_gamma = h->gammas.at(nf->gname); p.nrm_silu = nf->do_silu; p.nrm_scale = nf->scale;
+    }
     if (in.plane_scale > 0.f) {
         SVI_REQUIRE(in.plane_scale == p.in_scale, "conv %s: input planes carry scale %g, the layer expects %g", name.c_str(), in.plane_scale, p.in_scale);
         p.in = nullptr;
@@ -1694,14 +1813,44 @@
     return launch_rms_silu(in.p, out->p, (long)in.T * in.H * in.W, in.C, h->gammas.at(gname), do_silu, st);
 }
 
-svi_status res_block(svi_vae* h, const std::string& p, Tens* x, hipStream_t st) {
+static bool norm_fusable(svi_vae* h, const std::string& name, const Tens& in, float consumer_scale) {
+    if (h->dry || !(in.plane_scale > 0.f)) return false;
+    int To, Ho, Wo;
+    const ConvP p = conv_params(h->convs.at(name), in, 1, true, 1, 0, 0, false, &To, &Ho, &Wo);
+    return conv_norm_fusable(p, consumer_scale);
+}
+
+struct ResTap { unsigned short* mid_h; unsigned short* mid_l; float* mid_f32; };
+
+svi_status res_block(svi_vae* h, const std::string& p, Tens* x, hipStream_t st, const ResTap* tap = nullptr) {
     Tens n, hmid, out, skip;
     const bool has_sc = h->convs.count(p + "shortcut") > 0;
     if (has_sc) SVI_TRY(conv_layer(h, p + "shortcut", *x, &skip, st));
     SVI_TRY(norm_act(h, p + "residual.0.gamma", *x, &n, 1, st, planes_scale_for(h, p + "residual.2", p + "residual.0.gamma", *x)));
-    SVI_TRY(conv_layer(h, p + "residual.2", n, &hmid, st));
-    free_t(h, n);
-    SVI_TRY(norm_act(h, p + "residual.3.gamma", hmid, &n, 1, st, planes_scale_for(h, p + "residual.6", p + "residual.3.gamma", hmid)));
+    Tens mid_like = *x;
+    mid_like.C = h->convs.at(p + "residual.2").Cout;
+    const float s2 = planes_scale_for(h, p + "residual.6", p + "residual.3.gamma", mid_like);
+    const bool want_mid = tap && tap->mid_f32;
+    if (norm_fusable(h, p + "residual.2", n, s2)) {
+        const NormFuse nf{p + "residual.3.gamma", 1, s2, want_mid ? &hmid : nullptr};
+        Tens n2;
+        SVI_TRY(conv_layer(h, p + "residual.2", n, &n2, st, 1, true, 1, 0, 0, nullptr, false, &nf));
+        free_t(h, n);
+        n = n2;
+    } else {
+        SVI_TRY(conv_layer(h, p + "residual.2", n, &hmid, st));
+        free_t(h, n);
+        SVI_TRY(norm_act(h, p + "residual.3.gamma", hmid, &n, 1, st, s2));
+    }
+    if (tap && !h->dry) {
+        if (tap->mid_h) {
+            SVI_REQUIRE(n.plane_scale > 0.f, "svi_vae_res_block: the second convolution of '%s' does not read fp16 planes here", p.c_str());
+            const unsigned short* ph = reinterpret_cast<const unsigned short*>(n.p);
+            SVI_CHECK_HIP(hipMemcpyAsync(tap->mid_h, ph, (size_t)n.elems() * 2, hipMemcpyDeviceToDevice, st));
+            SVI_CHECK_HIP(hipMemcpyAsync(tap->mid_l, ph + n.elems(), (size_t)n.elems() * 2, hipMemcpyDeviceToDevice, st));
+        }
+        if (want_mid) SVI_CHECK_HIP(hipMemcpyAsync(tap->mid_f32, hmid.p, (size_t)hmid.elems() * 4, hipMemcpyDeviceToDevice, st));
+    }
     free_t(h, hmid);
     SVI_TRY(conv_layer(h, p + "residual.6", n, &out, st, 1, true, 1, 0, 0, has_sc ? &skip : x));
     free_t(h, n);
@@ -2371,6 +2520,27 @@
     return sized_run(h, [&] { return decode_graph(h, latents, video, T, hh, ww, nullptr, 0, 0, st); });
 }
 
+extern "C" svi_status svi_vae_res_block(svi_vae* h, const char* prefix, const float* x, float* out, int32_t T, int32_t H, int32_t W,
+                                        uint16_t* mid_h, uint16_t* mid_l, float* mid_f32, svi_stream stream) {
+    SVI_REQUIRE(h && prefix && x && out && T > 0 && H > 0 && W > 0 && !mid_h == !mid_l, "svi_vae_res_block: bad argument");
+    const std::string p(prefix);
+    SVI_REQUIRE(h->convs.count(p + "residual.2") && h->convs.count(p + "residual.6"), "svi_vae_res_block: '%s' is not a residual block", prefix);
+    SVI_REQUIRE(((uintptr_t)x | (uintptr_t)out | (uintptr_t)mid_h | (uintptr_t)mid_l | (uintptr_t)mid_f32) % 16 == 0, "svi_vae_res_block: tensors must be 16-byte aligned");
+    SVI_REQUIRE_DEVICE(h);
+    SVI_TRY(vae_prepare(h));
+    hipStream_t st = reinterpret_cast<hipStream_t>(stream);
+    const ResTap tap{mid_h, mid_l, mid_f32};
+    return sized_run(h, [&]() -> svi_status {
+        Tens t = alloc_t(h, T, H, W, h->convs.at(p + "residual.2").Cin);
+        NEED(t);
+        if (!h->dry) SVI_CHECK_HIP(hipMemcpyAsync(t.p, x, (size_t)t.elems() * 4, hipMemcpyDeviceToDevice, st));
+        SVI_TRY(res_block(h, p, &t, st, &tap));
+        if (!h->dry) SVI_CHECK_HIP(hipMemcpyAsync(out, t.p, (size_t)t.elems() * 4, hipMemcpyDeviceToDevice, st));
+        free_t(h, t);
+        return SVI_OK;
+    });
+}
+
 extern "C" svi_status svi_vae_split_plan(int32_t hh, int32_t ww, int32_t parts_h, int32_t parts_w, int32_t part, int32_t* out24) {
     SVI_REQUIRE(out24, "svi_vae_split_plan: null argument");
     SplitPlan pl{};
diff --git a/stable-video-infinity_amd/svi_hip/_lib.py b/stable-video-infinity_amd/svi_hip/_lib.py
--- a/stable-video-infinity_amd/svi_hip/_lib.py
+++ b/stable-video-infinity_amd/svi_hip/_lib.py
@@ -100,6 +100,8 @@
     ("svi_attention_plan", _i32, [_i32, _i32, _i32, _i32, C.POINTER(_i32)]),
     ("svi_vae_conv_plan", _i32, [_i32, _i32, _i32, _i32, _i32, _i32, C.POINTER(_i64)]),
     ("svi_vae_tile_order", _i32, [_i32, _i32, _i32, C.POINTER(_i64)]),
+    ("svi_vae_norm_fuse_plan", _i32, [_i32, _i32, _i32, _i32, C.POINTER(_i32)]),
+    ("svi_vae_res_block", _i32, [_vp, C.c_char_p, _vp, _vp, _i32, _i32, _i32, _vp, _vp, _vp, _vp]),
     ("svi_prof_enable", _i32, [_i32]),
     ("svi_prof_summary", _i32, [C.c_char_p, _i64]),
     ("svi_prof_select", _i32, [C.c_char_p]),
@@ -235,6 +237,12 @@
             "desc_bytes": out[6], "guard_bytes": out[7]}
 
 
+def vae_norm_fuse_plan(Cin: int, Cout: int, kt: int = 3, consumer_planes: bool = True) -> bool:
+    out = _i32(0)
+    check(lib().svi_vae_norm_fuse_plan(Cin, Cout, kt, 1 if consumer_planes else 0, C.byref(out)), "svi_vae_norm_fuse_plan")
+    return bool(out.value)
+
+
 def vae_tile_order(ord_T: int, ord_Lf: int, ord_G: int) -> list:
     out = (_i64 * (ord_T * ord_Lf))()
     check(lib().svi_vae_tile_order(ord_T, ord_Lf, ord_G, out), "svi_vae_tile_order")
diff --git a/stable-video-infinity_amd/svi_hip/vae.py b/stable-video-infinity_amd/svi_hip/vae.py
--- a/stable-video-infinity_amd/svi_hip/vae.py
+++ b/stable-video-infinity_amd/svi_hip/vae.py
@@ -148,6 +148,21 @@
         except Exception:
             pass
 
+    def res_block(self, prefix: str, x: torch.Tensor, planes: bool = False, mid_f32: bool = False) -> dict:
+        x = x.to(device="cuda", dtype=torch.float32).contiguous()
+        t, h, w, _ = x.shape
+        co = self._params[prefix + "residual.2.weight"].shape[0]
+        res = {"out": torch.empty((t, h, w, co), dtype=torch.float32, device=x.device)}
+        if planes:
+            res["mid_h"] = torch.zeros((t * h * w, co), dtype=torch.int16, device=x.device)
+            res["mid_l"] = torch.zeros((t * h * w, co), dtype=torch.int16, device=x.device)
+        if mid_f32:
+            res["mid"] = torch.zeros((t, h, w, co), dtype=torch.float32, device=x.device)
+        opt = lambda k: L.ptr(res[k]) if k in res else None
+        L.check(L.lib().svi_vae_res_block(self._h, prefix.encode(), L.ptr(x), L.ptr(res["out"]), t, h, w, opt("mid_h"), opt("mid_l"), opt("mid"),
+                                          L.current_stream()), "svi_vae_res_block")
+        return res
+
     def single_decode(self, hidden_state: torch.Tensor, device=None) -> torch.Tensor:
         z = hidden_state.to(device="cuda", dtype=torch.float32).contiguous()
         _, c, t, h, w = z.shape
```

New measurement: 1.014, median of 2. About the same (-0.0%).
